# ankur-maximos/Sparse_Matrix_with_Flops

Measured on AMD Instinct MI355X. Metric: SpGEMM GFLOP/s (2*intermediate_nnz/sec), C=A*A on 1M-row CSR, higher is better.
Workload: dtype f32; 1 GPU; synthetic power-law CSR 1048576^2, ~16 nnz/row, seed 43, C=A*A; m=1048576, nnzA=15623432, intermediate_nnz_P=238121643, nnzC=226057055, bytes_alg=3971793112, parallelism=single GPU

## Files before the change

### include/spgemm_hip.h

```cpp
#ifndef SPGEMM_HIP_H_
#define SPGEMM_HIP_H_

#include <stddef.h>

#ifdef __cplusplus
extern "C" {
#endif

#define SPGEMM_OK                0
#define SPGEMM_ERR_HIP           1
#define SPGEMM_ERR_ARG           2
#define SPGEMM_ERR_OVERFLOW      3
#define SPGEMM_ERR_NOMEM         4
#define SPGEMM_ERR_INPUT         5
#define SPGEMM_ERR_INTERNAL      6
#define SPGEMM_ERR_NODEVICE      7

#define SPGEMM_NBINS             9
#define SPGEMM_HV_LEN            9
#define SPGEMM_NKERNELS          21

typedef struct spgemm_handle spgemm_handle;

typedef struct spgemm_stats {
// ... 61 lines not shown
                       const int* dIA, const int* dJA, const float* dA, int nnzA,
                       const int* dIB, const int* dJB, const float* dB, int nnzB,
                       int m, int k, int n, const int* dIC, int* dJC, float* dC);

int hip_csr_row_flops(spgemm_handle* h, const int* dIA, const int* dJA, const int* dIB, int m,
                      int* dRowFlops, long long* total_flops);

int hip_gpuFlopsClassify(spgemm_handle* h,
                         const int* dIA, const int* dJA, const int* dIB,
                         int m, int k,
                         int** drowIds, int** dflops, int hv[SPGEMM_HV_LEN], int* hv_len,
                         long long* total_flops);

int hip_sgpuSpMM(spgemm_handle* h,
                 const int* dIA, const int* dJA, const float* dA, int nnzA,
                 const int* dIB, const int* dJB, const float* dB, int nnzB,
                 int m, int k, int n,
                 const int* drowIds, const int hv[SPGEMM_HV_LEN], const int* dflops,
                 int** dIC, int** dJC, float** dC, int* nnzC);

int hip_rmcl_prune(spgemm_handle* h, int m, const int* dIC, const int* dJC, float* dC,
                   int** dIN, int** dJN, float** dCN, int* nnzN);
int hip_rmcl_prune_n(spgemm_handle* h, int m, int nnz, const int* dIC, const int* dJC, const float* dC,
                     int** dIN, int** dJN, float** dCN, int* nnzN);
int hip_rmcl_expand_prune(spgemm_handle* h,
                          const int* dIA, const int* dJA, const float* dA, int nnzA,
                          const int* dIB, const int* dJB, const float* dB, int nnzB,
                          int m, int k, int n,
                          int** dIN, int** dJN, float** dCN, int* nnzN);
int hip_gpuRmclIter_device(spgemm_handle* h, int maxIter, int rows, int cols,
                           const int* dgI, const int* dgJ, const float* dgA, int gnnz,
                           const int* dtI, const int* dtJ, const float* dtA, int tnnz,
                           int** oI, int** oJ, float** oA, int* onnz);
int hip_gpuRmclIter(int maxIter, int rows, int cols,
                    const int* gIA, const int* gJA, const float* gA, int gnnz,
                    const int* tIA, const int* tJA, const float* tA, int tnnz,
                    int** oIA, int** oJA, float** oA, int* onnz);

#define SPGEMM_XCHG_AUTO  0
#define SPGEMM_XCHG_RCCL  1
#define SPGEMM_XCHG_PEER  2
#define SPGEMM_XCHG_HOST  3
#define SPGEMM_UNIQUE_ID_BYTES 128
typedef struct spgemm_group spgemm_group;
typedef struct spgemm_sharded spgemm_sharded;
int spgemm_hip_group_create(spgemm_group** g, int nshards, const int* devices, int transport);
int spgemm_hip_rccl_available(void);
int spgemm_hip_unique_id(void* id128);
int spgemm_hip_group_create_rank(spgemm_group** g, int nranks, int rank, int device, const void* id128);
int spgemm_hip_group_info(const spgemm_group* g, int* nranks, int* nlocal, int* transport);
int spgemm_hip_group_destroy(spgemm_group* g);

int hip_sharded_spmm_create(spgemm_group* g, const int* IA, const int* JA, const float* A, int nnzA,
                            const int* IB, const int* JB, const float* B, int nnzB, int m, int k, int n,
                            spgemm_sharded** job);
int hip_sharded_spmm_step(spgemm_sharded* job, int gather, long long* nnzC, long long* totalP);
int hip_sharded_spmm_result(spgemm_sharded* job, int local_shard, int** IC, int** JC, float** C, int* nnzC, int* rows);
int hip_sharded_spmm_info(spgemm_sharded* job, int* ends, float* ms_compute, float* ms_exchange);
spgemm_handle* hip_sharded_spmm_handle(spgemm_sharded* job, int local_shard);
int hip_sharded_spmm_destroy(spgemm_sharded* job);

int hip_gpuRmclIter_sharded(spgemm_group* g, int maxIter, int rows, int cols,
                            const int* gIA, const int* gJA, const float* gA, int gnnz,
                            const int* tIA, const int* tJA, const float* tA, int tnnz,
                            int** oIA, int** oJA, float** oA, int* onnz);

typedef struct spgemm_sharded_rmcl spgemm_sharded_rmcl;
int hip_sharded_rmcl_create(spgemm_group* g, int rows, int cols, const int* gIA, const int* gJA, const float* gA, int gnnz,
                            const int* tIA, const int* tJA, const float* tA, int tnnz, spgemm_sharded_rmcl** job);
int hip_sharded_rmcl_run(spgemm_sharded_rmcl* job, int maxIter, int* nnz);
int hip_sharded_rmcl_continue(spgemm_sharded_rmcl* job, int iters, int* nnz);
int hip_sharded_rmcl_result(spgemm_sharded_rmcl* job, int local_shard, int** oIA, int** oJA, float** oA, int* onnz);
int hip_sharded_rmcl_iter_nnz(const spgemm_sharded_rmcl* job, long long* out, int cap);
int hip_sharded_rmcl_info(const spgemm_sharded_rmcl* job, int* ends);
int hip_sharded_rmcl_destroy(spgemm_sharded_rmcl* job);

int spgemm_hip_handle_device(const spgemm_handle* h);

int spgemm_hip_rmcl_devices_used(void);

int spgemm_hip_debug_fail_next(spgemm_handle* h, int count);

int spgemm_hip_debug_bigrow_paths(spgemm_handle* h, int* direct_rows, int* fallback_rows, int* rehit_cap, int* region_ints);

#define SPGEMM_COO_DEDUPE         1
#define SPGEMM_COO_SELF_LOOPS     2
#define SPGEMM_COO_ROW_NORMALISE  4
#define SPGEMM_COO_ABS            8
int hip_coo_to_csr(spgemm_handle* h, int rows, int cols, int nnz, const int* dRow, const int* dCol, const float* dVal,
                   int flags, int** dIA, int** dJA, float** dA, int* nnzOut);

#define SPGEMM_EDGES_ONE_BASED 1
#define SPGEMM_EDGES_TRANSPOSE 2
typedef struct spgemm_edge_stats {
  long long lines;
  long long first_bad_line;
  int entries, slow_lines;
  float ms_upload, ms_split, ms_parse, ms_slow, ms_total;
} spgemm_edge_stats;

int hip_edge_text_header(const char* text, size_t nbytes, int* rows, int* cols, int* declared,
                         int* one_based, int* symmetric, size_t* data_offset);
int hip_parse_edge_lines(spgemm_handle* h, const char* dText, size_t nbytes, int declared, int flags,
                         int** dRow, int** dCol, float** dVal, int* entries, spgemm_edge_stats* st);
int hip_parse_edge_text (spgemm_handle* h, const char* text,  size_t nbytes, int declared, int flags,
                         int** dRow, int** dCol, float** dVal, int* entries, spgemm_edge_stats* st);
int hip_read_edge_file  (spgemm_handle* h, const char* path, int isTrans, int cooFlags, int* rows, int* cols,
                         int** dIA, int** dJA, float** dA, int* nnz, spgemm_edge_stats* st);

#define SPGEMM_STATS_LEN 13
int hip_flopsStats(spgemm_handle* h, const int* dIA, const int* dJA, const int* dIB, int m, int stats[SPGEMM_STATS_LEN]);

#define SPGEMM_NNZ_STATS_LEN 18
int hip_nnzStats(spgemm_handle* h, const int* dIA, int m, int stats[SPGEMM_NNZ_STATS_LEN]);

typedef struct spgemm_bin_report {
  int rows;
  int rows_differ;
  int first_bad_row;
  double max_rel_err;
} spgemm_bin_report;
int hip_resultsComparison(int m, int n, const int* hIC, const int* hJC, const float* hC,
                          const int* rIC, const int* rJC, const float* rC,
                          const int hv[SPGEMM_HV_LEN], int hv_len, const int* hqueue, double rel,
                          spgemm_bin_report report[SPGEMM_HV_LEN - 1]);

int hip_csr_sort_rows(spgemm_handle* h, int m, const int* dIC, int* dJC, float* dC);

int hip_csr_permute(spgemm_handle* h, int m, int n, int nnz, const int* dIA, const int* dJA, const float* dA,
                    const int* dRowSrc, const int* dColMap, int** dIB, int** dJB, float** dB);
int hip_csr_permute_f64(spgemm_handle* h, int m, int n, int nnz, const int* dIA, const int* dJA, const double* dA,
                        const int* dRowSrc, const int* dColMap, int** dIB, int** dJB, double** dB);

int hip_permutation_transpose(spgemm_handle* h, int len, const int* dP, int* dPt);

int hip_csr_row_descending_permutation(spgemm_handle* h, int m, const int* dIA, int** dP);

int hip_csr_transpose(spgemm_handle* h, int m, int n, int nnz, const int* dIA, const int* dJA, const float* dA,
                      int** dIT, int** dJT, float** dAT);
int hip_csr_transpose_f64(spgemm_handle* h, int m, int n, int nnz, const int* dIA, const int* dJA, const double* dA,
                          int** dIT, int** dJT, double** dAT);

typedef struct spgemm_csr_diff {
  int       rows_len_differ;
  int       first_len_row;
  long long only_a, only_b;
  int       first_only_row;
  long long beyond;
  int       first_beyond_row;
  double    max_abs_err;
  double    max_rel_err;
  double    max_abs_only_a, max_abs_only_b;
  double    sum_sq;
} spgemm_csr_diff;
int hip_csr_diff(spgemm_handle* h, int m, int n,
                 const int* dIA, const int* dJA, const float* dA, int nnzA,
                 const int* dIB, const int* dJB, const float* dB, int nnzB,
                 double rel_tol, double abs_tol, spgemm_csr_diff* out);
int hip_csr_diff_f64(spgemm_handle* h, int m, int n,
                     const int* dIA, const int* dJA, const double* dA, int nnzA,
                     const int* dIB, const int* dJB, const double* dB, int nnzB,
                     double rel_tol, double abs_tol, spgemm_csr_diff* out);

int hip_csr_differsStats(spgemm_handle* h, int m, const int* dIA, const int* dIB,
                         const float* percents, int npercents, int* counts);
int hip_csr_differsStats_f64(spgemm_handle* h, int m, const int* dIA, const int* dIB,
// ... 72 lines not shown
```

### sparse_matrix_with_flops_amd/csrc/spgemm_device.hpp

```cpp
#pragma once
#include <hip/hip_runtime.h>
#include <stdint.h>
#include <type_traits>

namespace smf {

#ifdef SMF_ABLATE
__device__ int g_ablate = 0;
#define ABL(bit) (g_ablate & (bit))
__device__ __forceinline__ void smf_or(int*, int) {}
__device__ __forceinline__ void smf_or(unsigned* p, unsigned v) { atomicOr(p, v); }
#define atomicOr(p, v) smf_or((p), (v))
#else
#define ABL(bit) 0
#endif

constexpr int WAVE = 64;

template <class T> __device__ __forceinline__ void st_out(T* p, T v) {
#ifdef SMF_PLAIN_STORES
  *p = v;
#else
  __builtin_nontemporal_store(v, p);
#endif
// ... 27 lines not shown
  while (lg < 12 + NSUB - 1 && (f >> (lg + 1)) != 0) ++lg;
  return SLOT_BIG0 + (NSUB - 1 - (lg - 12));
}
__host__ __device__ __forceinline__ int last_slot_of_bin(int b) {
  return b < 5 ? b : b == 5 ? SLOT_H1B : b == 6 ? SLOT_H4B : b == 7 ? SLOT_H8 : NSLOTS - 1;
}

constexpr int ERRF_TABLE_FULL = 1;
constexpr int ERRF_COUNT_MISMATCH = 2;

__device__ __forceinline__ int lane_id() { return (int)__lane_id(); }

__device__ __forceinline__ unsigned long long ballot64(bool pred) { return __builtin_amdgcn_ballot_w64(pred); }

__device__ __forceinline__ int mask_rank(unsigned long long mask) {
  return (int)__builtin_amdgcn_mbcnt_hi((unsigned)(mask >> 32), __builtin_amdgcn_mbcnt_lo((unsigned)mask, 0u));
}

#define SMF_DPP(v, ctrl, rowmask, ident) __builtin_amdgcn_update_dpp((ident), (v), (ctrl), (rowmask), 0xf, false)

__device__ __forceinline__ int wave_incl_add(int v) {
  v += SMF_DPP(v, 0x111, 0xf, 0);
  v += SMF_DPP(v, 0x112, 0xf, 0);
  v += SMF_DPP(v, 0x114, 0xf, 0);
  v += SMF_DPP(v, 0x118, 0xf, 0);
  v += SMF_DPP(v, 0x142, 0xa, 0);
  v += SMF_DPP(v, 0x143, 0xc, 0);
  return v;
}

__device__ __forceinline__ int wave_incl_max(int v) {
  v = max(v, SMF_DPP(v, 0x111, 0xf, 0));
  v = max(v, SMF_DPP(v, 0x112, 0xf, 0));
  v = max(v, SMF_DPP(v, 0x114, 0xf, 0));
  v = max(v, SMF_DPP(v, 0x118, 0xf, 0));
  v = max(v, SMF_DPP(v, 0x142, 0xa, 0));
  v = max(v, SMF_DPP(v, 0x143, 0xc, 0));
  return v;
}

__device__ __forceinline__ int wave_sum(int v) { return __builtin_amdgcn_readlane(wave_incl_add(v), 63); }

__device__ __forceinline__ unsigned long long wave_sum_u64(unsigned long long v) {
#pragma unroll
  for (int d = 32; d >= 1; d >>= 1) v += __shfl_xor(v, d, 64);
  return v;
}

__device__ __forceinline__ void wave_lds_sync() {
  __builtin_amdgcn_fence(__ATOMIC_ACQ_REL, "wavefront");
  __builtin_amdgcn_s_waitcnt(0xc07f);
  __builtin_amdgcn_wave_barrier();
}

__device__ __forceinline__ int next_pow2_clamped(int x, int lo, int hi) {
  int p = lo;
  while (p < x && p < hi) p <<= 1;
  return p;
}

__device__ __forceinline__ int log2_pow2(int p) { return 31 - __clz(p); }

template <int MULT = 2>
__device__ __forceinline__ int table_size(int items, int lo, int hi) {
  return items >= hi / MULT ? hi : next_pow2_clamped(MULT * items, lo, hi);
}

__device__ __forceinline__ int hash_insert(int* keys, int size, int shift, int c, bool* is_new, int* err) {
  unsigned h = ((unsigned)c * 2654435761u) >> shift;
  const unsigned mask = (unsigned)size - 1u;
  *is_new = false;
  for (int probe = 0; probe < size; ++probe) {
    const int old = atomicCAS(&keys[h], EMPTY_KEY, c);
    if (old == EMPTY_KEY) { *is_new = true; return (int)h; }
    if (old == c) return (int)h;
    h = (h + 1u) & mask;
  }
  atomicOr(err, ERRF_TABLE_FULL);
  return 0;
}

constexpr int DUMMY_KEY = (int)0x80000000;

template <bool POW2 = true, int U>
__device__ __forceinline__ int hash_insert_multi(int* keys, int size, int shift, const bool (&act)[U],
                                                 const int (&col)[U], int* dummy, int* err) {
  char* const base = reinterpret_cast<char*>(keys);
  const int dumB = (int)(reinterpret_cast<char*>(dummy) - base);
  const int maskB = size * 4 - 1;
  int hB[U];
  int claimed = 0;
#pragma unroll
  for (int u = 0; u < U; ++u) {
    const unsigned hv = (unsigned)col[u] * 2654435761u;
    const unsigned h = POW2 ? hv >> shift : __umulhi(hv, (unsigned)size);
    hB[u] = act[u] ? (int)(h * 4u) : dumB;
  }
  int probe = 0;
  for (;;) {
    int old[U];
#pragma unroll
    for (int u = 0; u < U; ++u) old[u] = atomicCAS(reinterpret_cast<int*>(base + hB[u]), EMPTY_KEY, col[u]);
    ++probe;
    int pendBits = 0;
#pragma unroll
    for (int u = 0; u < U; ++u) {
      claimed += old[u] == EMPTY_KEY ? 1 : 0;
      const bool adv = hB[u] != dumB && old[u] != EMPTY_KEY && old[u] != col[u];
      const int nh = POW2 ? ((hB[u] + probe * 4) & maskB) : (hB[u] + 4 == size * 4 ? 0 : hB[u] + 4);
      hB[u] = adv ? nh : dumB;
      pendBits |= hB[u] ^ dumB;
    }
    if (ballot64(pendBits != 0) == 0ull) break;
    if (probe >= size) { atomicOr(err, ERRF_TABLE_FULL); break; }
  }
  return claimed;
}

typedef unsigned long long slot_t;
constexpr slot_t EMPTY_SLOT = 0x00000000FFFFFFFFull;
constexpr slot_t DUMMY_SLOT = 0x0000000080000000ull;
__device__ __forceinline__ slot_t make_slot(int col, float v) {
  return (slot_t)(unsigned)col | ((slot_t)__float_as_uint(v) << 32);
}
__device__ __forceinline__ int slot_key(slot_t sl) { return (int)(unsigned)sl; }
__device__ __forceinline__ float slot_val(slot_t sl) { return __uint_as_float((unsigned)(sl >> 32)); }
__device__ __forceinline__ float* slot_val_ptr(slot_t* tab, unsigned i) { return reinterpret_cast<float*>(tab + i) + 1; }

__device__ __forceinline__ void hash_accum(slot_t* tab, int size, int shift, int c, float v, int* err) {
  unsigned h = ((unsigned)c * 2654435761u) >> shift;
  const unsigned mask = (unsigned)size - 1u;
  const slot_t mine = make_slot(c, v);
  for (int probe = 0; probe < size; ++probe) {
    const slot_t old = atomicCAS(&tab[h], EMPTY_SLOT, mine);
    if (old == EMPTY_SLOT) return;
    if (slot_key(old) == c) { atomicAdd(slot_val_ptr(tab, h), v); return; }
    h = (h + 1u) & mask;
  }
  atomicOr(err, ERRF_TABLE_FULL);
}

template <bool POW2 = true, int U>
__device__ __forceinline__ void hash_accum_multi(slot_t* tab, int size, int shift, const bool (&act)[U],
                                                 const int (&col)[U], const float (&val)[U], slot_t* dummy, int* err) {
  char* const base = reinterpret_cast<char*>(tab);
  const int dumB = (int)(reinterpret_cast<char*>(dummy) - base);
  const int maskB = size * 8 - 1, sizeB = size * 8;
  int hB[U], stepB[U], dupB[U];
  slot_t mine[U];
#pragma unroll
  for (int u = 0; u < U; ++u) {
    const unsigned hv = (unsigned)col[u] * 2654435761u;
    const unsigned h = POW2 ? hv >> shift : __umulhi(hv, (unsigned)size);
    stepB[u] = POW2 ? 0 : (int)((0x2f2b29251f1d1713ull >> (((hv >> 7) & 7u) * 8u)) & 0xffu) * 8;
    hB[u] = act[u] ? (int)(h * 8u) : dumB;
    dupB[u] = dumB;
    mine[u] = make_slot(col[u], val[u]);
  }
  int probe = 0;
  for (;;) {
    slot_t old[U];
#pragma unroll
    for (int u = 0; u < U; ++u) old[u] = atomicCAS(reinterpret_cast<slot_t*>(base + hB[u]), EMPTY_SLOT, mine[u]);
    ++probe;
    int pendBits = 0;
#pragma unroll
    for (int u = 0; u < U; ++u) {
      const bool pend = hB[u] != dumB;
      const bool same = pend && slot_key(old[u]) == col[u];
      const bool adv = pend && old[u] != EMPTY_SLOT && slot_key(old[u]) != col[u];
      dupB[u] = same ? hB[u] : dupB[u];
      int nh;
      if (POW2) nh = (hB[u] + probe * 8) & maskB;
      else { nh = hB[u] + stepB[u]; nh = nh >= sizeB ? nh - sizeB : nh; }
      hB[u] = adv ? nh : dumB;
      pendBits |= hB[u] ^ dumB;
    }
    if (ballot64(pendBits != 0) == 0ull) break;
    if (probe >= size) { atomicOr(err, ERRF_TABLE_FULL); break; }
  }
#pragma unroll
  for (int u = 0; u < U; ++u)
    if (dupB[u] != dumB) atomicAdd(reinterpret_cast<float*>(base + dupB[u] + 4), val[u]);
}

template <int U>
__device__ __forceinline__ void lds_fadd_multi(float* acc, const int (&idx)[U], const bool (&ok)[U], const float (&v)[U],
                                               int* dummy) {
  int* ia = reinterpret_cast<int*>(acc);
  int old[U];
  bool pend[U];
#pragma unroll
  for (int u = 0; u < U; ++u) { pend[u] = ok[u]; old[u] = ia[ok[u] ? idx[u] : 0]; }
  for (;;) {
    int got[U];
#pragma unroll
    for (int u = 0; u < U; ++u)
      got[u] = atomicCAS(pend[u] ? &ia[idx[u]] : dummy, old[u], __float_as_int(__int_as_float(old[u]) + v[u]));
    bool more = false;
#pragma unroll
    for (int u = 0; u < U; ++u) {
      pend[u] = pend[u] && got[u] != old[u];
      old[u] = got[u];
      more = more || pend[u];
    }
    if (ballot64(more) == 0ull) break;
  }
}

template <int NW> struct InsChunk { static constexpr int value = NW == 1 ? 1 : 0; };
template <int CH, int R>
__device__ __forceinline__ int hash_insert_chunked(int* keys, int size, int shift, const bool (&act)[R], const int (&col)[R],
                                                   int* dummy, int* err) {
  if constexpr (CH <= 0 || CH >= R) return hash_insert_multi(keys, size, shift, act, col, dummy, err);
  else {
    int claimed = 0;
#pragma unroll
    for (int c0 = 0; c0 < R; c0 += CH) {
      bool a_[CH]; int c_[CH];
#pragma unroll
      for (int u = 0; u < CH; ++u) { a_[u] = c0 + u < R ? act[c0 + u < R ? c0 + u : 0] : false; c_[u] = col[c0 + u < R ? c0 + u : 0]; }
      if (CH == 1 && ballot64(a_[0]) == 0ull) continue;
      claimed += hash_insert_multi(keys, size, shift, a_, c_, dummy, err);
    }
    return claimed;
  }
}
template <int CH, int R>
__device__ __forceinline__ void hash_accum_chunked(slot_t* tab, int size, int shift, const bool (&act)[R], const int (&col)[R],
                                                   const float (&val)[R], slot_t* dummy, int* err) {
  if constexpr (CH <= 0 || CH >= R) hash_accum_multi(tab, size, shift, act, col, val, dummy, err);
  else {
#pragma unroll
    for (int c0 = 0; c0 < R; c0 += CH) {
      bool a_[CH]; int c_[CH]; float v_[CH];
#pragma unroll
      for (int u = 0; u < CH; ++u) {
        const int i = c0 + u < R ? c0 + u : 0;
        a_[u] = c0 + u < R ? act[i] : false; c_[u] = col[i]; v_[u] = val[i];
      }
      if (CH == 1 && ballot64(a_[0]) == 0ull) continue;
      hash_accum_multi(tab, size, shift, a_, c_, v_, dummy, err);
    }
  }
}

__device__ __forceinline__ void clear_slots(slot_t* tab, int size, int tid, int nthreads) {
  for (int i = tid * 2; i < size; i += nthreads * 2) *reinterpret_cast<ulonglong2*>(tab + i) = make_ulonglong2(EMPTY_SLOT, EMPTY_SLOT);
}

__device__ __forceinline__ void clear_table(int* keys, float* vals, int size, int tid, int nthreads) {
  const int4 ek = make_int4(EMPTY_KEY, EMPTY_KEY, EMPTY_KEY, EMPTY_KEY);
  const float4 zv = make_float4(0.f, 0.f, 0.f, 0.f);
  for (int i = tid * 4; i < size; i += nthreads * 4) {
    *reinterpret_cast<int4*>(keys + i) = ek;
    if (vals) *reinterpret_cast<float4*>(vals + i) = zv;
  }
}

template <int MAXSTEPS>
__device__ __forceinline__ void emit_claimed(const slot_t* tab, int base, int per, int* emitted,
                                             int outLo, int outHi, int* __restrict__ JC, float* __restrict__ C) {
  const int lane = lane_id();
  slot_t sl[MAXSTEPS];
  int cnt = 0;
#pragma unroll
  for (int sidx = 0; sidx < MAXSTEPS; ++sidx) {
    sl[sidx] = sidx * WAVE < per ? tab[base + sidx * WAVE + lane] : EMPTY_SLOT;
    cnt += __popcll(ballot64(slot_key(sl[sidx]) != EMPTY_KEY));
  }
  int pos = 0;
  if (lane == 0) pos = atomicAdd(emitted, cnt);
  pos = __builtin_amdgcn_readfirstlane(pos);
  int* const JCrow = JC + outLo;
  float* const Crow = C + outLo;
  const unsigned lim = (unsigned)(outHi - outLo);
#pragma unroll
  for (int sidx = 0; sidx < MAXSTEPS; ++sidx) {
    const bool occ = slot_key(sl[sidx]) != EMPTY_KEY;
    const unsigned long long mk = ballot64(occ);
    const unsigned o = (unsigned)(pos + mask_rank(mk));
    if (occ && o < lim) { st_out(JCrow + o, slot_key(sl[sidx])); st_out(Crow + o, slot_val(sl[sidx])); }
    pos += __popcll(mk);
  }
}

__device__ __forceinline__ float rmcl_threshold(float avg, float mx) {
  float ret = (float)(0.90 * avg * (1 - 2 * (mx - avg)));
  ret = (float)((ret > 1.0e-7) ? ret : 1.0e-7);
  ret = (ret > mx) ? mx : ret;
  return ret;
}

template <class Op>
__device__ __forceinline__ float row16_allreduce(float v, Op op) {
  v = op(v, __int_as_float(SMF_DPP(__float_as_int(v), 0xB1, 0xf, 0)));
  v = op(v, __int_as_float(SMF_DPP(__float_as_int(v), 0x4E, 0xf, 0)));
  v = op(v, __int_as_float(SMF_DPP(__float_as_int(v), 0x141, 0xf, 0)));
  v = op(v, __int_as_float(SMF_DPP(__float_as_int(v), 0x140, 0xf, 0)));
  return v;
}
template <int L, class Op>
__device__ __forceinline__ float rowL_allreduce(float v, Op op) {
  static_assert(L == 16 || L == 64, "16-lane groups or whole waves");
  v = row16_allreduce(v, op);
  if (L == 64) {
// ... 677 lines not shown
    const int sIncl = wave_incl_add(ntg), lIncl = wave_incl_add(lug);
    const int S = __builtin_amdgcn_readlane(sIncl, 63);
    const int total = S + __builtin_amdgcn_readlane(lIncl, 63);
    int tIncl = 0, lpIncl = 0, gLPv = 0, shortSum = 0;
    if (num) {
      gLPv = lane < NW ? num->gLP[lane] : 0;
      tIncl = wave_incl_add(gT);
      lpIncl = wave_incl_add(gLPv);
      shortSum = __builtin_amdgcn_readlane(tIncl, 63);
    }
    for (int u = __builtin_amdgcn_readfirstlane(w); u < total;) {
      int unext = 0;
      if (lane == 0) unext = atomicAdd(&st.claim, 1);
      if (u < S) {
        const int g = __popcll(ballot64(sIncl <= u));
        const int t = u - (__builtin_amdgcn_readlane(sIncl, g) - __builtin_amdgcn_readlane(ntg, g));
        const int T = __builtin_amdgcn_readlane(gT, g), ns = __builtin_amdgcn_readlane(gNS, g);
        unsigned long long W[U];
        int base[U];
#pragma unroll
        for (int uu = 0; uu < U; ++uu) {
          const int r = min(t * U + uu, WAVE - 1);
          W[uu] = st.marks[g][r];
          base[uu] = st.wpre[g][r];
        }
        const int p0 = num ? chunkBase + (__builtin_amdgcn_readlane(tIncl, g) - T) + t * U * WAVE : -1;
        short_trip<U, NEED_VAL, 16>(reinterpret_cast<const char*>(st.rec[g]), T, ns, t * U, W, base, JB, VB, f, p0);
      } else {
        const int ul = u - S;
        const int g = __popcll(ballot64(lIncl <= ul));
        const int ug = ul - (__builtin_amdgcn_readlane(lIncl, g) - __builtin_amdgcn_readlane(lug, g));
        const int nl = __builtin_amdgcn_readlane(gNL, g);
        const int uex = lane < nl ? st.rec[g][WAVE - 1 - lane].w : 0x7fffffff;
        const int k = __popcll(ballot64(uex <= ug)) - 1;
        const int4 r4 = st.rec[g][WAVE - 1 - k];
        const int p0 = num ? chunkBase + shortSum + (__builtin_amdgcn_readlane(lpIncl, g) - __builtin_amdgcn_readlane(gLPv, g)) +
                                 num->lpro[g][k] + (ug - r4.w) * UP
                           : -1;
        long_trip<U, NEED_VAL>(r4.x, r4.z, __int_as_float(r4.y), (ug - r4.w) * UP, JB, VB, f, p0);
      }
      u = __builtin_amdgcn_readfirstlane(unext);
    }
    __builtin_amdgcn_s_waitcnt(0xc07f);
    if (num) chunkBase += shortSum + __builtin_amdgcn_readlane(lpIncl, 63);
    __syncthreads();
  }
}

template <int R>
__device__ __forceinline__ int next_row(int* ctr, int* slot, int prev) {
  if (R > 1 && prev >= 0 && (prev + 1) % R != 0) return prev + 1;
  if (threadIdx.x == 0) *slot = atomicAdd(ctr, R);
  __syncthreads();
  const int q = *slot;
  __syncthreads();
  return q;
}
__device__ __forceinline__ int next_row(int* ctr, int* slot) { return next_row<1>(ctr, slot, -1); }

struct RowMeta { int row, as, ae, x0, x1, x2; };

__device__ __forceinline__ RowMeta load_meta_sym(const int* rows, int q, int count, const int* IA, const int* rowFlops) {
  RowMeta mtd{0, 0, 0, 0, 0, 0};
  if (q < count) { mtd.row = rows[q]; mtd.as = IA[mtd.row]; mtd.ae = IA[mtd.row + 1]; mtd.x0 = rowFlops[mtd.row]; }
  return mtd;
}
__device__ __forceinline__ RowMeta load_meta_num(const int* rows, int q, int count, const int* IA, const int* IC,
                                                 const int* rowFlops = nullptr) {
  RowMeta mtd{0, 0, 0, 0, 0, 0};
  if (q < count) {
    mtd.row = rows[q]; mtd.as = IA[mtd.row]; mtd.ae = IA[mtd.row + 1]; mtd.x0 = IC[mtd.row]; mtd.x1 = IC[mtd.row + 1];
    if (rowFlops) mtd.x2 = rowFlops[mtd.row];
  }
  return mtd;
}

__device__ __forceinline__ PreA load_pre(const RowMeta& mtd, const int2* SBL, const float* VA, bool needVal) {
  PreA p{0, 0, 0.f, true};
  const int ap = mtd.as + lane_id();
  if (ap < mtd.ae) { const int2 sbl = SBL[ap]; p.bs = sbl.x; p.len = sbl.y; if (needVal) p.a = VA[ap]; }
  return p;
}

template <int NW, int TBL, int U>
__global__ __launch_bounds__(WAVE * NW) void k_sym_hash(const int* __restrict__ binPtr, int bin,
                                                         const int* __restrict__ rowIds,
                                                         const int* __restrict__ IA, const int2* __restrict__ SBL,
                                                         const int* __restrict__ JB,
                                                         const int* __restrict__ rowFlops, int* __restrict__ IC,
                                                         int* __restrict__ err, int* __restrict__ qctr) {
  __shared__ __attribute__((aligned(16))) int keys[TBL];
  __shared__ typename WalkSel<NW>::type st;
  __shared__ int cnt_s;
  __shared__ int qslot;
  const int tid = threadIdx.x, lane = lane_id();
  if (tid < WAVE) st.dummy[tid] = DUMMY_SLOT;
  int first = binPtr[bin], count = binPtr[bin + 1] - first;
  constexpr int QB = NW >= 8 ? 2 : 4;
  int stride = (int)gridDim.x;
  if (NW == 1) {
    const XcdRange xr = xcd_range(count);
    first += xr.lo; count = xr.hi - xr.lo; stride = xr.nb;
  }
  const int* rows = rowIds + first;
  int q = NW > 1 ? next_row<QB>(qctr, &qslot, -1) : (int)(blockIdx.x >> 3);
  RowMeta cur = load_meta_sym(rows, q, count, IA, rowFlops);
  RowMeta nxt = NW == 1 ? load_meta_sym(rows, q + stride, count, IA, rowFlops) : RowMeta{0, 0, 0, 0, 0, 0};
  PreA pc = NW == 1 ? load_pre(cur, SBL, nullptr, false) : PreA{0, 0, 0.f, false};
  while (q < count) {
    int qn;
    PreA pn{0, 0, 0.f, false};
    RowMeta nn{0, 0, 0, 0, 0};
    if (NW == 1) {
      qn = q + stride;
      nn = load_meta_sym(rows, qn + stride, count, IA, rowFlops);
      pn = load_pre(nxt, SBL, nullptr, false);
    } else {
      qn = next_row<QB>(qctr, &qslot, q);
      nxt = load_meta_sym(rows, qn, count, IA, rowFlops);
    }
    const int size = table_size<4>(cur.x0, 64, TBL);
    const int shift = 32 - log2_pow2(size);
    clear_table(keys, nullptr, size, tid, WAVE * NW);
    if (tid == 0) cnt_s = 0;
    __syncthreads();
    int mine = 0;
    for_each_product<NW, U, false>(st, cur.as, cur.ae, SBL, nullptr, JB, nullptr,
                                   [&](const auto& act, const auto& col, const auto& val, int) {
      mine += hash_insert_chunked<InsChunk<NW>::value>(keys, size, shift, act, col, reinterpret_cast<int*>(&st.dummy[lane_id()]), err);
    }, pc, err);
    const int ws = wave_sum(mine);
    if (NW == 1) {
      if (lane == 0) IC[cur.row] = ws;
    } else {
      if (lane == 0 && ws) atomicAdd(&cnt_s, ws);
      __syncthreads();
      if (tid == 0) IC[cur.row] = cnt_s;
    }
    __syncthreads();
    cur = nxt;
    if (NW == 1) { nxt = nn; pc = pn; }
    q = qn;
  }
}

template <int NW, int TBL, int U, int PRUNE = 0>
__global__ __launch_bounds__(WAVE * NW) void k_num_hash(const int* __restrict__ binPtr, int bin,
                                                         const int* __restrict__ rowIds,
                                                         const int* __restrict__ IA, const int2* __restrict__ SBL,
                                                         const float* __restrict__ VA,
                                                         const int* __restrict__ JB,
                                                         const float* __restrict__ VB,
                                                         const int* __restrict__ IC, int* __restrict__ JC,
                                                         float* __restrict__ C, int* __restrict__ err,
                                                         int* __restrict__ qctr, const int* __restrict__ rowFlops,
                                                         int* __restrict__ pcnt) {
  __shared__ __attribute__((aligned(16))) slot_t tab[TBL];
  __shared__ PruneShared<NW> ps;
  __shared__ typename WalkSel<NW>::type st;
  __shared__ int qslot;
  __shared__ int emitted;
  const int tid = threadIdx.x;
  if (tid < WAVE) st.dummy[tid] = DUMMY_SLOT;
  constexpr int T = WAVE * NW;
  int first = binPtr[bin], count = binPtr[bin + 1] - first;
  constexpr int QB = NW >= 8 ? 2 : 4;
  int stride = (int)gridDim.x;
  if (NW == 1) {
    const XcdRange xr = xcd_range(count);
    first += xr.lo; count = xr.hi - xr.lo; stride = xr.nb;
  }
  const int* rows = rowIds + first;
  int q = NW > 1 ? next_row<QB>(qctr, &qslot, -1) : (int)(blockIdx.x >> 3);
  const int* const rf = rowFlops;
  RowMeta cur = load_meta_num(rows, q, count, IA, IC, rf);
  RowMeta nxt = NW == 1 ? load_meta_num(rows, q + stride, count, IA, IC, rf) : RowMeta{0, 0, 0, 0, 0, 0};
  PreA pc = NW == 1 ? load_pre(cur, SBL, VA, true) : PreA{0, 0, 0.f, false};
  while (q < count) {
    int qn;
    PreA pn{0, 0, 0.f, false};
    RowMeta nn{0, 0, 0, 0, 0};
    if (NW == 1) {
      qn = q + stride;
      nn = load_meta_num(rows, qn + stride, count, IA, IC, rf);
      pn = load_pre(nxt, SBL, VA, true);
    } else {
      qn = next_row<QB>(qctr, &qslot, q);
      nxt = load_meta_num(rows, qn, count, IA, IC, rf);
    }
    const int off = cur.x0;
    const int want = cur.x1 - off;
    if (NW == 1 && PRUNE == 1 && want == cur.x2 && want <= TBL) {
      for_each_product<NW, U, true>(st, cur.as, cur.ae, SBL, VA, JB, VB,
                                    [&](const auto& act, const auto& col, const auto& val, int p0) {
        constexpr int R = (int)(sizeof(col) / sizeof(col[0]));
#pragma unroll
        for (int u = 0; u < R; ++u) {
          const unsigned o = (unsigned)(p0 + u * WAVE + lane_id());
          if (act[u] && o < (unsigned)want) tab[o] = make_slot(col[u], val[u]);
        }
      }, pc, err);
      wave_lds_sync();
      int nocc;
      const int kept = prune_emit_group<64>(tab, (want + 63) & ~63, want, false, true, lane_id(), JC + off, C + off, &nocc);
      if (lane_id() == 0) pcnt[cur.row] = kept;
      wave_lds_sync();
      cur = nxt;
      nxt = nn; pc = pn;
      q = qn;
      continue;
    }
    if (NW == 1 && PRUNE == 0 && want == cur.x2) {
      int* const JCrow = JC + off;
      float* const Crow = C + off;
      for_each_product<NW, U, true>(st, cur.as, cur.ae, SBL, VA, JB, VB,
                                    [&](const auto& act, const auto& col, const auto& val, int p0) {
        constexpr int R = (int)(sizeof(col) / sizeof(col[0]));
#pragma unroll
        for (int u = 0; u < R; ++u) {
          const unsigned o = (unsigned)(p0 + u * WAVE + lane_id());
          if (act[u] && o < (unsigned)want) { st_out(JCrow + o, col[u]); st_out(Crow + o, val[u]); }
        }
      }, pc, err);
      cur = nxt;
      if (NW == 1) { nxt = nn; pc = pn; }
      q = qn;
// ... 565 lines not shown
      clear_slots(sh.tab, size, tid, T);
      if (tid == 0) sh.emitted = 0;
      __syncthreads();
      {
        const int* const lg = rlLog + cur.ls;
        const unsigned mask = (unsigned)size - 1u;
        for (int i = tid; i < lc; i += T) {
          const int c = lg[i];
          const slot_t mine = make_slot(c, -0.0f);
          unsigned h = ((unsigned)c * 2654435761u) >> shift;
          for (int probe = 0; probe < size; ++probe) {
            const slot_t old = atomicCAS(&sh.tab[h], EMPTY_SLOT, mine);
            if (old == EMPTY_SLOT || slot_key(old) == c) break;
            h = (h + 1u) & mask;
          }
        }
      }
      __syncthreads();
      int* const JCrow = JC + outBase;
      float* const Crow = C + outBase;
      const unsigned lim = (unsigned)max(want, 0);
      for_each_product<NW, BD_U, true>(sh.st, as, ae, SBL, VA, JB, VB,
                                       [&](const bool (&act)[BD_U], const int (&col)[BD_U], const float (&val)[BD_U], int) {
        char* const base = reinterpret_cast<char*>(sh.tab);
        const int dumB = (int)(reinterpret_cast<char*>(&sh.st.dummy[lane]) - base);
        const int maskB = size * 8 - 1;
        int hB[BD_U], hitB[BD_U];
        bool miss[BD_U];
#pragma unroll
        for (int u = 0; u < BD_U; ++u) {
          const unsigned h = ((unsigned)col[u] * 2654435761u) >> shift;
          hB[u] = act[u] ? (int)(h * 8u) : dumB;
          hitB[u] = dumB;
          miss[u] = false;
        }
        for (int probe = 0;;) {
          int key[BD_U];
#pragma unroll
          for (int u = 0; u < BD_U; ++u) key[u] = *reinterpret_cast<const int*>(base + hB[u]);
          ++probe;
          int pendBits = 0;
#pragma unroll
          for (int u = 0; u < BD_U; ++u) {
            const bool pend = hB[u] != dumB;
            const bool hit = pend && key[u] == col[u];
            const bool emp = pend && key[u] == EMPTY_KEY;
            hitB[u] = hit ? hB[u] : hitB[u];
            miss[u] = miss[u] || emp;
            hB[u] = (pend && !hit && !emp) ? ((hB[u] + 8) & maskB) : dumB;
            pendBits |= hB[u] ^ dumB;
          }
          if (ballot64(pendBits != 0) == 0ull) break;
          if (probe >= size) { atomicOr(err, ERRF_TABLE_FULL); break; }
        }
#pragma unroll
        for (int u = 0; u < BD_U; ++u)
          if (hitB[u] != dumB) atomicAdd(reinterpret_cast<float*>(base + hitB[u] + 4), val[u]);
        unsigned long long mk[BD_U];
        int tot = 0;
#pragma unroll
        for (int u = 0; u < BD_U; ++u) { mk[u] = ballot64(miss[u]); tot += __popcll(mk[u]); }
        if (tot) {
          int pos = 0;
          if (lane == 0) pos = atomicAdd(&sh.emitted, tot);
          pos = __builtin_amdgcn_readfirstlane(pos);
#pragma unroll
          for (int u = 0; u < BD_U; ++u) {
            const unsigned o = (unsigned)(pos + mask_rank(mk[u]));
            if (miss[u] && o < lim) { st_out(JCrow + o, col[u]); st_out(Crow + o, val[u]); }
            pos += __popcll(mk[u]);
          }
        }
      });
      emit_claimed<S / NW / WAVE>(sh.tab, w * per, per, &sh.emitted, outBase, outEnd, JC, C);
      __syncthreads();
      if (tid == 0 && sh.emitted != want) atomicOr(err, ERRF_COUNT_MISMATCH);
      __syncthreads();
    }
    cur = nxt;
    q = qn;
  }
}

constexpr int SCAN_THREADS = 1024;
constexpr int SCAN_ITEMS = 4;
constexpr int SCAN_TILE = SCAN_THREADS * SCAN_ITEMS;

__global__ __launch_bounds__(SCAN_THREADS) void k_scan_tile_sums(int m, const int* __restrict__ IC,
                                                                  unsigned long long* __restrict__ tileSum) {
  __shared__ unsigned long long red[16];
  const int tid = threadIdx.x, lane = lane_id(), w = tid >> 6;
  const int base = blockIdx.x * SCAN_TILE + tid * SCAN_ITEMS;
  unsigned long long s = 0;
#pragma unroll
  for (int i = 0; i < SCAN_ITEMS; ++i) if (base + i < m) s += (unsigned)IC[base + i];
  s = wave_sum_u64(s);
  if (lane == 0) red[w] = s;
  __syncthreads();
  if (tid == 0) { unsigned long long t = 0; for (int i = 0; i < 16; ++i) t += red[i]; tileSum[blockIdx.x] = t; }
}

__global__ __launch_bounds__(1024) void k_scan_tiles(int ntiles, unsigned long long* __restrict__ tileSum,
                                                      unsigned long long* __restrict__ total) {
  __shared__ unsigned long long wsum[16];
  __shared__ unsigned long long running;
  const int tid = threadIdx.x, lane = lane_id(), w = tid >> 6;
  if (tid == 0) running = 0;
  __syncthreads();
  for (int t0 = 0; t0 < ntiles; t0 += 1024) {
    const int t = t0 + tid;
    const unsigned long long v = t < ntiles ? tileSum[t] : 0ull;
    unsigned long long incl = v;
#pragma unroll
    for (int d = 1; d < 64; d <<= 1) { const unsigned long long o = __shfl_up(incl, d, 64); if (lane >= d) incl += o; }
    if (lane == 63) wsum[w] = incl;
    __syncthreads();
    unsigned long long woff = 0, tot = 0;
    for (int i = 0; i < 16; ++i) { const unsigned long long s = wsum[i]; tot += s; if (i < w) woff += s; }
    const unsigned long long run = running;
    if (t < ntiles) tileSum[t] = run + woff + incl - v;
    __syncthreads();
    if (tid == 0) running = run + tot;
    __syncthreads();
  }
  if (tid == 0) *total = running;
}

__global__ __launch_bounds__(SCAN_THREADS) void k_scan_apply(int m, int* __restrict__ IC,
                                                              const unsigned long long* __restrict__ tileOff,
                                                              const unsigned long long* __restrict__ total, int clampTotal) {
  __shared__ int wsum[16];
  const int tid = threadIdx.x, lane = lane_id(), w = tid >> 6;
  const int base = blockIdx.x * SCAN_TILE + tid * SCAN_ITEMS;
  int v[SCAN_ITEMS];
  int s = 0;
#pragma unroll
  for (int i = 0; i < SCAN_ITEMS; ++i) { v[i] = base + i < m ? IC[base + i] : 0; s += v[i]; }
  const int incl = wave_incl_add(s);
  if (lane == 63) wsum[w] = incl;
  __syncthreads();
  int woff = 0;
  for (int i = 0; i < w; ++i) woff += wsum[i];
  int run = (int)tileOff[blockIdx.x] + woff + incl - s;
#pragma unroll
  for (int i = 0; i < SCAN_ITEMS; ++i) { if (base + i < m) IC[base + i] = run; run += v[i]; }
  if (blockIdx.x == 0 && tid == 0) {
    const unsigned long long t = *total;
    IC[m] = (clampTotal && t > 0x7fffffffULL) ? 0x7fffffff : (int)(unsigned)t;
  }
}

__global__ void k_gather_flops(int m, const int* __restrict__ rowIds, const int* __restrict__ rowFlops,
                               int* __restrict__ out) {
  const int q = blockIdx.x * blockDim.x + threadIdx.x;
  if (q < m) out[q] = rowFlops[rowIds[q]];
}

constexpr int SORT_MAX = 4096;
template <class V>
__global__ __launch_bounds__(256) void k_sort_rows(int m, const int* __restrict__ IC, int* __restrict__ JC,
                                                    V* __restrict__ C, int* __restrict__ longUnsorted) {
  __shared__ int sk[SORT_MAX];
  __shared__ V sv[SORT_MAX];
  __shared__ int unsorted;
  const int tid = threadIdx.x;
  for (int row = blockIdx.x; row < m; row += gridDim.x) {
// ... 272 lines not shown
```

### sparse_matrix_with_flops_amd/csrc/spgemm_hip.hip

```cpp
#include "spgemm_device.hpp"
#include "spgemm_f64_device.hpp"
#include "chain_device.hpp"
#include "../../include/spgemm_hip.h"

#include <algorithm>
#include <array>
#include <chrono>
#include <climits>
#include <cmath>
#include <cstdarg>
#include <cstdio>
#include <cstdlib>
#include <cstring>
#include <map>
#include <mutex>
#include <sys/mman.h>
#include <thread>
#include <type_traits>
#include <vector>

using namespace smf;

static_assert(NBINS == SPGEMM_NBINS, "bin count of the kernels and of the C ABI differ");
#ifdef SMF_ABLATE
// ... 68 lines not shown
    return e;
  }
  hipError_t release(void* p) {
    if (!p) return hipSuccess;
    if (check) (void)hipDeviceSynchronize();
    Blk blk{0, 0};
    {
      std::lock_guard<std::mutex> lk(mu);
      auto it = live.find(p);
      if (it == live.end()) return hipFree(p);
      blk = it->second;
      live.erase(it);
      if (cached_bytes + blk.size <= kMaxCached) {
        free_blocks[blk.dev].emplace(blk.size, p);
        cached_bytes += blk.size;
        return hipSuccess;
      }
    }
    return hipFree(p);
  }
  void trim(int dev) {
    std::lock_guard<std::mutex> lk(mu);
    auto& fb = free_blocks[dev];
    for (auto& kv : fb) { cached_bytes -= kv.first; (void)hipFree(kv.second); }
    fb.clear();
  }
  size_t cached_on(int dev) {
    std::lock_guard<std::mutex> lk(mu);
    size_t t = 0;
    for (auto& kv : free_blocks[dev]) t += kv.first;
    return t;
  }
};
DevPool& pool() { static DevPool* p = new DevPool(); return *p; }

template <class T>
struct DevBuf {
  T* p = nullptr;
  DevBuf() = default;
  DevBuf(DevBuf&& o) noexcept : p(o.release()) {}
  DevBuf& operator=(DevBuf&& o) noexcept { if (this != &o) { reset(); p = o.release(); } return *this; }
  ~DevBuf() { reset(); }
  hipError_t alloc(size_t n) { reset(); return pool().alloc((void**)&p, sizeof(T) * n); }
  void reset() { pool().release(p); p = nullptr; }
  T* release() { T* q = p; p = nullptr; return q; }
  operator T*() const { return p; }
};

struct CsrView {
  const int* I; const int* J; const float* V; int nnz;
  const int* len = nullptr; const int2* se = nullptr;
};

struct DevCSR {
  DevBuf<int> I, J; DevBuf<float> V; DevBuf<int> len; DevBuf<int2> se;
  int rows = 0, cols = 0, nnz = 0;
  bool packed() const { return !len; }
  CsrView view() const { return {I, J, V, nnz, len, se}; }
  hipError_t alloc_entries(long long n) {
    const hipError_t e = J.alloc((size_t)std::max(n, 1ll));
    return e != hipSuccess ? e : V.alloc((size_t)std::max(n, 1ll));
  }
  void reset() { *this = DevCSR(); }
  void give(int** oI, int** oJ, float** oV, int* onnz) {
    *oI = I.release(); *oJ = J.release(); *oV = V.release(); *onnz = nnz;
    reset();
  }
};

static int drained(hipStream_t s, int rc) {
  if (rc) (void)hipStreamSynchronize(s);
  return rc;
}
struct Retired {
  DevCSR m;
  void park(DevCSR&& operand) { m = std::move(operand); }
};
}

struct HostMirror {
  int binPtr[NBINS + 1];
  int err;
  int scratch2[4];
  alignas(128) int qctr[9 * 32];
  alignas(128) int qpad_;
  int slotBase[NSLOTS + 1];
  unsigned long long totalP;
  unsigned long long nnzC64;
  unsigned long long kept64;
  unsigned long long cutTotal;
  int nBatches;
  alignas(128) int chainTicket;
  alignas(128) int chainPad_;
  alignas(128) int fbBin[2];
  alignas(128) int fbPad_;
};

struct spgemm_handle {
  int device = 0;
  int numCU = 256;
  hipStream_t stream = nullptr;
  hipEvent_t ev[6] = {nullptr, nullptr, nullptr, nullptr, nullptr, nullptr};
  int cap_m = -1;
  int* rowFlops = nullptr;
  unsigned char* binId = nullptr;
  int* blockHist = nullptr;
  int* blockOff = nullptr;
  int* rowIds = nullptr;
  unsigned long long* tileSum = nullptr;
  unsigned long long* blockP = nullptr;
  int2* sbl = nullptr;
  int* batchStart = nullptr;
  unsigned long long* chainWords = nullptr;
  int pathMode = 0;
  int chainCfg = 0;
  long long cap_nnz = -1;
  HostMirror* dsmall = nullptr;
  HostMirror* hsmall = nullptr;
  HostMirror mirror;
  const int* cur_rowIds = nullptr;
  int sym_m = -1;
  hipEvent_t kev[2 * SPGEMM_NKERNELS];
  bool kused[SPGEMM_NKERNELS];
  unsigned ktiming = 0;
  hipEvent_t evMid = nullptr;
  HostMirror* hmid = nullptr;
  static constexpr int NSIDE = 4;
  hipStream_t side[NSIDE] = {nullptr, nullptr, nullptr, nullptr};
  hipEvent_t fork_ev = nullptr;
  hipEvent_t join_ev[NSIDE] = {nullptr, nullptr, nullptr, nullptr};
  bool serial = true;
  int U = 2;
  unsigned* bigBitmaps = nullptr;
  int bm_cap = 0;
  int2* spill = nullptr;
  int spill_blocks = 0;
  int bhCap = BH_CAP;
  int bhMargin = 125;
  bool bigDirect = true;
  int bdCfg = 1;
  int bdMinRows = 0;
  int rlRegionEnv = 0;
  int2* rlMeta = nullptr;
  int rl_rows = 0;
  int* rlLog = nullptr;
  int rl_region = 0;
  int* bigFallback = nullptr;
  bool bdLogged = false;
  bool bdRan = false;
  int h1sym = 32;
  int h1num = 24;
  spgemm_stats stats;
  spgemm_host_api_stats host_api = {};
  int failNext = 0;
  int prev_m = -1;
  unsigned long long prev_P = 0;
  long long prev_nnzC = -1;
};

static std::mutex g_count_mu;
static std::map<int, int> g_handles_on;

struct WsBlock { void** ptr; size_t bytes; };
static std::array<WsBlock, 10> ws_blocks(spgemm_handle* h, size_t cap) {
  const size_t nblk = (cap + K1_THREADS - 1) / K1_THREADS;
  const size_t ntile = (cap + 1 + SCAN_TILE - 1) / SCAN_TILE + 1;
  return {{{(void**)&h->rowFlops, sizeof(int) * cap},
           {(void**)&h->binId, cap},
           {(void**)&h->blockHist, sizeof(int) * nblk * NSLOTS},
           {(void**)&h->blockOff, sizeof(int) * nblk * NSLOTS},
           {(void**)&h->rowIds, sizeof(int) * cap},
           {(void**)&h->tileSum, sizeof(unsigned long long) * ntile},
           {(void**)&h->blockP, sizeof(unsigned long long) * nblk},
           {(void**)&h->bigFallback, sizeof(int) * cap},
           {(void**)&h->batchStart, sizeof(int) * (3 * cap + 64)},
           {(void**)&h->chainWords, sizeof(unsigned long long) * (3 * cap + 64)}}};
}

static int ws_free(spgemm_handle* h) {
  for (const WsBlock& b : ws_blocks(h, 0)) { hipFree(*b.ptr); *b.ptr = nullptr; }
  h->cap_m = -1;
  return SPGEMM_OK;
}

static int ws_ensure_entries(spgemm_handle* h, long long nnzA) {
  if (nnzA <= h->cap_nnz) return SPGEMM_OK;
  hipFree(h->sbl);
  h->sbl = nullptr; h->cap_nnz = -1;
  const long long cap = nnzA + nnzA / 8 + 1024;
  HIPCHK(hipMalloc((void**)&h->sbl, sizeof(int2) * (size_t)cap));
  h->cap_nnz = cap;
  return SPGEMM_OK;
}

static int ws_ensure(spgemm_handle* h, int m) {
  if (m <= h->cap_m) return SPGEMM_OK;
  ws_free(h);
  const size_t cap = (size_t)m + (size_t)m / 8 + 1024;
  for (const WsBlock& b : ws_blocks(h, cap)) HIPCHK(hipMalloc(b.ptr, b.bytes));
  h->cap_m = (int)std::min<size_t>(cap, 0x7fffffff);
  return SPGEMM_OK;
}

template <class F>
static auto with_bd_cfg(int cfg, F f) {
  typedef std::integral_constant<int, 4> W4; typedef std::integral_constant<int, 8> W8; typedef std::integral_constant<int, 16> W16;
  typedef std::integral_constant<int, 4096> S4; typedef std::integral_constant<int, 8192> S8;
  switch (cfg) {
    case 0: return f(W4(), S4());
    case 1: return f(W8(), S4());
    case 2: return f(W4(), S8());
    case 4: return f(W16(), S4());
    default: return f(W8(), S8());
  }
}
static int bd_cap_of(int cfg) { return bd_cap(cfg == 2 || cfg == 3 ? 8192 : 4096); }

static void env_int(const char* name, int lo, int hi, int* field) {
  if (const char* e = getenv(name)) { const int v = atoi(e); if (v >= lo && v <= hi) *field = v; }
}

extern "C" int spgemm_hip_device_count(int* count) {
  if (!count) return fail(SPGEMM_ERR_ARG, "count is null");
  int n = 0;
  hipError_t e = hipGetDeviceCount(&n);
  if (e != hipSuccess) { *count = 0; return fail(SPGEMM_ERR_NODEVICE, "hipGetDeviceCount: %s", hipGetErrorString(e)); }
  *count = n;
  return SPGEMM_OK;
}

extern "C" int spgemm_hip_create(spgemm_handle** out, int device) {
  if (!out) return fail(SPGEMM_ERR_ARG, "handle out-pointer is null");
  *out = nullptr;
  int n = 0;
  if (hipGetDeviceCount(&n) != hipSuccess || n <= 0)
    return fail(SPGEMM_ERR_NODEVICE, "no HIP device visible: libspgemm_hip has no CPU fallback");
  if (device < 0 || device >= n) return fail(SPGEMM_ERR_ARG, "device %d out of range [0,%d)", device, n);
  HIPCHK(hipSetDevice(device));
  spgemm_handle* h = new spgemm_handle();
  h->device = device;
  hipDeviceProp_t prop;
  HIPCHK(hipGetDeviceProperties(&prop, device));
  h->numCU = prop.multiProcessorCount > 0 ? prop.multiProcessorCount : 256;
  HIPCHK(hipStreamCreateWithFlags(&h->stream, hipStreamNonBlocking));
  for (auto& e : h->ev) HIPCHK(hipEventCreate(&e));
  for (auto& e : h->kev) HIPCHK(hipEventCreate(&e));
  for (auto& u : h->kused) u = false;
  { const char* e = getenv("SPGEMM_CONCURRENT"); h->serial = !(e && e[0] == '1'); }
#ifdef SMF_ABLATE
  { int v = 0; env_int("SPGEMM_ABLATE", INT_MIN, INT_MAX, &v); HIPCHK(hipMemcpyToSymbol(HIP_SYMBOL(smf::g_ablate), &v, sizeof(int))); }
#endif
  env_int("SPGEMM_H1SYM", 1, 32, &h->h1sym);
  env_int("SPGEMM_H1NUM", 1, 32, &h->h1num);
  env_int("SPGEMM_BHMARGIN", 10, 400, &h->bhMargin);
  env_int("SPGEMM_BHCAP", 1024, BH_CAP_MAX, &h->bhCap);
  { int v = 1; env_int("SPGEMM_BIGDIRECT", 0, 1, &v); h->bigDirect = v != 0; }
  env_int("SPGEMM_BD_CFG", 0, 4, &h->bdCfg);
  h->bdMinRows = h->numCU;
  env_int("SPGEMM_BD_MINROWS", 1, 1 << 30, &h->bdMinRows);
  env_int("SPGEMM_RLREGION", 64, 1 << 24, &h->rlRegionEnv);
  env_int("SPGEMM_PATH", 0, 2, &h->pathMode);
  env_int("SPGEMM_CHAIN_CFG", INT_MIN, INT_MAX, &h->chainCfg);
  { int u = h->U; env_int("SPGEMM_U", 2, 8, &u); if (u == 2 || u == 4 || u == 8) h->U = u; }
  for (auto& st : h->side) {
    if (h->serial) st = h->stream;
    else HIPCHK(hipStreamCreateWithFlags(&st, hipStreamNonBlocking));
  }
  HIPCHK(hipEventCreateWithFlags(&h->fork_ev, hipEventDisableTiming));
  for (auto& e : h->join_ev) HIPCHK(hipEventCreateWithFlags(&e, hipEventDisableTiming));
  HIPCHK(hipMalloc((void**)&h->dsmall, sizeof(HostMirror)));
  HIPCHK(hipHostMalloc((void**)&h->hsmall, sizeof(HostMirror), hipHostMallocDefault));
  HIPCHK(hipHostMalloc((void**)&h->hmid, sizeof(HostMirror), hipHostMallocDefault));
  HIPCHK(hipEventCreateWithFlags(&h->evMid, hipEventDisableTiming));
  { const char* e = getenv("SPGEMM_KTIMING"); if (e) h->ktiming = (unsigned)strtoul(e, nullptr, 0); }
  memset(&h->stats, 0, sizeof(h->stats));
  { std::lock_guard<std::mutex> lk(g_count_mu); ++g_handles_on[device]; }
  HIPCHK(hipFuncSetAttribute((const void*)k_sym_big<false>, hipFuncAttributeMaxDynamicSharedMemorySize, (int)sizeof(BigSymShared)));
  HIPCHK(hipFuncSetAttribute((const void*)k_sym_big<true>, hipFuncAttributeMaxDynamicSharedMemorySize, (int)sizeof(BigSymShared)));
  HIPCHK(with_bd_cfg(h->bdCfg, [&](auto nw, auto slots) {
    return hipFuncSetAttribute((const void*)k_num_bigdirect<nw, slots>, hipFuncAttributeMaxDynamicSharedMemorySize,
                               (int)sizeof(BigDirectShared<nw, slots>)); }));
  HIPCHK(hipFuncSetAttribute((const void*)k_num_big, hipFuncAttributeMaxDynamicSharedMemorySize, (int)sizeof(BigNumShared)));
  HIPCHK(hipFuncSetAttribute((const void*)k_num_bighash, hipFuncAttributeMaxDynamicSharedMemorySize, (int)sizeof(BigHashShared)));
  *out = h;
  return SPGEMM_OK;
}

extern "C" int spgemm_hip_destroy(spgemm_handle* h) {
  if (!h) return SPGEMM_OK;
  hipSetDevice(h->device);
  if (h->stream) hipStreamSynchronize(h->stream);
  for (auto& st : h->side) if (st && st != h->stream) { hipStreamSynchronize(st); hipStreamDestroy(st); }
  ws_free(h);
  hipFree(h->bigBitmaps);
  hipFree(h->spill);
  hipFree(h->rlMeta);
  hipFree(h->rlLog);
  hipFree(h->sbl);
  hipFree(h->dsmall);
  hipHostFree(h->hsmall);
  hipHostFree(h->hmid);
  if (h->evMid) hipEventDestroy(h->evMid);
  for (auto& e : h->ev) if (e) hipEventDestroy(e);
  for (auto& e : h->kev) if (e) hipEventDestroy(e);
  if (h->fork_ev) hipEventDestroy(h->fork_ev);
  for (auto& e : h->join_ev) if (e) hipEventDestroy(e);
  if (h->stream) hipStreamDestroy(h->stream);
  bool last = false;
  { std::lock_guard<std::mutex> lk(g_count_mu); last = --g_handles_on[h->device] <= 0; }
  if (last) pool().trim(h->device);
  delete h;
  return SPGEMM_OK;
}

extern "C" int spgemm_hip_get_stats(const spgemm_handle* h, spgemm_stats* out) {
  if (!h || !out) return fail(SPGEMM_ERR_ARG, "null argument");
  *out = h->stats;
  return SPGEMM_OK;
}

extern "C" void* spgemm_hip_stream(spgemm_handle* h) { return h ? (void*)h->stream : nullptr; }

extern "C" int spgemm_hip_handle_device(const spgemm_handle* h) { return h ? h->device : -1; }

extern "C" int spgemm_hip_debug_bigrow_paths(spgemm_handle* h, int* direct_rows, int* fallback_rows, int* rehit_cap, int* region_ints) {
  if (!h || !direct_rows || !fallback_rows || !rehit_cap || !region_ints) return fail(SPGEMM_ERR_ARG, "null argument");
  const int nbig = h->mirror.binPtr[NBINS] - h->mirror.binPtr[NBINS - 1];
  *fallback_rows = h->bdRan ? h->mirror.fbBin[1] : nbig;
  *direct_rows = nbig - *fallback_rows;
  *rehit_cap = bd_cap_of(h->bdCfg);
  *region_ints = h->rl_region;
  return SPGEMM_OK;
}

extern "C" int spgemm_hip_debug_fail_next(spgemm_handle* h, int count) {
  if (!h) return fail(SPGEMM_ERR_ARG, "null handle");
  h->failNext = count;
  return SPGEMM_OK;
}

extern "C" int spgemm_hip_set_kernel_timing(spgemm_handle* h, unsigned mask) {
  if (!h) return fail(SPGEMM_ERR_ARG, "null handle");
  h->ktiming = mask;
  return SPGEMM_OK;
}

static std::mutex g_default_mu;
static spgemm_handle* g_default = nullptr;
static int default_handle(spgemm_handle** out) {
  std::lock_guard<std::mutex> lk(g_default_mu);
  if (!g_default) CHK(spgemm_hip_create(&g_default, 0));
  *out = g_default;
  return SPGEMM_OK;
}

extern "C" int spgemm_hip_malloc(void** dptr, size_t bytes) {
  if (!dptr) return fail(SPGEMM_ERR_ARG, "dptr is null");
  *dptr = nullptr;
  HIPCHK(pool().alloc(dptr, bytes ? bytes : 1));
  return SPGEMM_OK;
}
extern "C" int spgemm_hip_pool_cached_bytes(int device, size_t* bytes) {
  if (!bytes) return fail(SPGEMM_ERR_ARG, "bytes is null");
  *bytes = pool().cached_on(device);
  return SPGEMM_OK;
}
extern "C" int spgemm_hip_pool_trim(int device) {
  int n = 0;
  if (hipGetDeviceCount(&n) != hipSuccess || device < 0 || device >= n) return fail(SPGEMM_ERR_ARG, "device %d out of range", device);
  int cur = 0;
  const bool had = hipGetDevice(&cur) == hipSuccess;
  HIPCHK(hipSetDevice(device));
  pool().trim(device);
  if (had) (void)hipSetDevice(cur);
  return SPGEMM_OK;
}
extern "C" int spgemm_hip_free(void* dptr) {
  HIPCHK(pool().release(dptr));
  return SPGEMM_OK;
}
struct CopyJob { void* host; void* dev; size_t bytes; };
static int copy_pageable(int dev, const CopyJob* jobs, int njobs, bool toDevice);
static constexpr size_t kLaneCopyMin = size_t(8) << 20;
static int device_of(const void* dptr) {
  hipPointerAttribute_t a;
  if (hipPointerGetAttributes(&a, dptr) == hipSuccess) return a.device;
  (void)hipGetLastError();
  int dev = 0;
  (void)hipGetDevice(&dev);
  return dev;
}

extern "C" int spgemm_hip_memcpy_h2d(void* dst, const void* src, size_t bytes) {
  if (bytes && (!dst || !src)) return fail(SPGEMM_ERR_ARG, "null pointer in h2d copy");
  if (bytes >= kLaneCopyMin) {
    const CopyJob j{const_cast<void*>(src), dst, bytes};
    return copy_pageable(device_of(dst), &j, 1, true);
  }
  if (bytes) HIPCHK(hipMemcpy(dst, src, bytes, hipMemcpyHostToDevice));
  return SPGEMM_OK;
}
extern "C" int spgemm_hip_memcpy_d2h(void* dst, const void* src, size_t bytes) {
  if (bytes && (!dst || !src)) return fail(SPGEMM_ERR_ARG, "null pointer in d2h copy");
  if (bytes >= kLaneCopyMin) {
    const CopyJob j{dst, const_cast<void*>(src), bytes};
    return copy_pageable(device_of(src), &j, 1, false);
  }
  if (bytes) HIPCHK(hipMemcpy(dst, src, bytes, hipMemcpyDeviceToHost));
  return SPGEMM_OK;
}

extern "C" int spgemm_hip_memcpy_d2d(void* dst, const void* src, size_t bytes) {
  if (bytes && (!dst || !src)) return fail(SPGEMM_ERR_ARG, "null pointer in d2d copy");
  if (bytes) HIPCHK(hipMemcpy(dst, src, bytes, hipMemcpyDeviceToDevice));
// ... 16 lines not shown
    "k_num_hash<1,1024>", "k_num_hash<4,4096>", "k_num_hash<8,8192>", "k_num_big", "k_num_bighash", "k_cut(3 launches)",
    "k_chain", "k_wbatch<sym>", "k_wbatch<num>"};
extern "C" const char* spgemm_hip_kernel_name(int id) { return (id >= 0 && id < SPGEMM_NKERNELS) ? kKernelNames[id] : ""; }

struct KTimer {
  spgemm_handle* h; int id; hipStream_t s; bool on;
  KTimer(spgemm_handle* h_, int id_, hipStream_t s_ = nullptr)
      : h(h_), id(id_), s(s_ ? s_ : h_->stream), on((h_->ktiming >> id_) & 1u) {
    if (on) { hipEventRecord(h->kev[2 * id], s); h->kused[id] = true; }
  }
  ~KTimer() { if (on) hipEventRecord(h->kev[2 * id + 1], s); }
};

static void collect_kernel_times(spgemm_handle* h, bool reset) {
  for (int i = 0; i < SPGEMM_NKERNELS; ++i) {
    if (reset) h->stats.ms_kernel[i] = 0.f;
    if (h->kused[i]) { float ms = 0.f; if (hipEventElapsedTime(&ms, h->kev[2 * i], h->kev[2 * i + 1]) == hipSuccess) h->stats.ms_kernel[i] = ms; }
    h->kused[i] = false;
  }
}

static void fork_streams(spgemm_handle* h) {
  if (h->serial) return;
  hipEventRecord(h->fork_ev, h->stream);
  for (auto& st : h->side) hipStreamWaitEvent(st, h->fork_ev, 0);
}
static void join_streams(spgemm_handle* h) {
  if (h->serial) return;
  for (int i = 0; i < spgemm_handle::NSIDE; ++i) {
    hipEventRecord(h->join_ev[i], h->side[i]);
    hipStreamWaitEvent(h->stream, h->join_ev[i], 0);
  }
}

#define LAUNCH_U(KERN, NW, TBL, grid, block, st, ...)                                              \
  do {                                                                                             \
    if (h->U == 8) hipLaunchKernelGGL((KERN<NW, TBL, 8>), grid, block, 0, st, __VA_ARGS__);        \
    else if (h->U == 4) hipLaunchKernelGGL((KERN<NW, TBL, 4>), grid, block, 0, st, __VA_ARGS__);   \
    else hipLaunchKernelGGL((KERN<NW, TBL, 2>), grid, block, 0, st, __VA_ARGS__);                  \
  } while (0)

template <class F>
static void with_prune_arg(const int* pcnt, int pmode, F f) {
  if (pcnt && pmode == 2) f(std::integral_constant<int, 2>());
  else if (pcnt) f(std::integral_constant<int, 1>());
  else f(std::integral_constant<int, 0>());
}

#define LAUNCH_NUM(NW, TBL, grid, block, st, ...)                                                                  \
  with_prune_arg(pcnt, pmode, [&](auto prune) {                                                                    \
    if constexpr (prune != 0) hipLaunchKernelGGL((k_num_hash<NW, TBL, 2, prune>), grid, block, 0, st, __VA_ARGS__, pcnt); \
    else LAUNCH_U(k_num_hash, NW, TBL, grid, block, st, __VA_ARGS__, (int*)nullptr);                               \
  })

static int launch_classify(spgemm_handle* h, const int* dIA, const int* dJA, const int* dIB, int m, long long nnzA, int* dIC,
                           const int2* dIBse = nullptr) {
  const int nblk = cdiv(m, K1_THREADS);
  clear_stale_hip_error();
  HIPCHK(hipMemsetAsync(h->dsmall, 0, sizeof(HostMirror), h->stream));
  if (nnzA >= 0) CHK(ws_ensure_entries(h, nnzA));
  if (m > 0) {
    { KTimer t(h, SPGEMM_K_ROW_FLOPS);
      int2* const sbl = nnzA >= 0 ? h->sbl : (int2*)nullptr;
      const int cap = (int)std::max(nnzA, 0ll);
      if (dIBse) hipLaunchKernelGGL(k_row_flops<true>, dim3(nblk), dim3(K1_THREADS), 0, h->stream, m, dIA, dJA, dIB, dIBse,
                                    sbl, cap, h->rowFlops, h->binId, h->blockHist, h->blockP, dIC);
      else hipLaunchKernelGGL(k_row_flops<false>, dim3(nblk), dim3(K1_THREADS), 0, h->stream, m, dIA, dJA, dIB, dIBse,
                              sbl, cap, h->rowFlops, h->binId, h->blockHist, h->blockP, dIC); }
    { KTimer t(h, SPGEMM_K_BIN_SCAN);
      hipLaunchKernelGGL(k_bin_scan, dim3(1), dim3(1024), 0, h->stream, nblk, h->blockHist, h->blockOff,
                         h->dsmall->binPtr, h->dsmall->slotBase, h->blockP, &h->dsmall->totalP); }
    { KTimer t(h, SPGEMM_K_SCATTER);
      hipLaunchKernelGGL(k_scatter_rows, dim3(nblk), dim3(K1_THREADS), 0, h->stream, m, h->binId, h->blockOff,
                         h->dsmall->slotBase, h->rowIds); }
  }
  HIPCHK(hipGetLastError());
  return SPGEMM_OK;
}

static int launch_symbolic(spgemm_handle* h, const int* dIA, const int* dJB,
                           int m, int n, const int* rowIds, int* dIC, int minBin = 0, bool skipH1A = false, bool logBig = false) {
  const int2* sbl = h->sbl;
  h->bdLogged = logBig && h->bigDirect && n > BIG_WC && m > 0;
  if (m <= 0) return SPGEMM_OK;
  clear_stale_hip_error();
  const int* bp = h->dsmall->binPtr;
  int* err = &h->dsmall->err;
  int* qc = h->dsmall->qctr;
  const int cu = h->numCU;
  fork_streams(h);
  { hipStream_t st = h->side[3]; KTimer t(h, SPGEMM_K_SYM_BIG, st);
    if (h->bdLogged)
      hipLaunchKernelGGL(k_sym_big<true>, dim3(clampi(m, 1, cu)), dim3(BIG_THREADS), sizeof(BigSymShared), st, bp, 8,
                         rowIds, dIA, sbl, dJB, n, dIC, h->bigBitmaps, h->bm_cap, qc + 0 * 32,
                         h->rlMeta, h->rlLog ? h->rl_rows : 0, h->rlLog, h->rl_region, bd_cap_of(h->bdCfg), h->bigFallback,
                         &h->dsmall->fbBin[1]);
    else
      hipLaunchKernelGGL(k_sym_big<false>, dim3(clampi(m, 1, cu)), dim3(BIG_THREADS), sizeof(BigSymShared), st, bp, 8,
                         rowIds, dIA, sbl, dJB, n, dIC, h->bigBitmaps, h->bm_cap, qc + 0 * 32,
                         (int2*)nullptr, 0, (int*)nullptr, 0, 0, (int*)nullptr, (int*)nullptr); }
  if (minBin <= 7) { hipStream_t st = h->side[2]; KTimer t(h, SPGEMM_K_SYM_HASH8, st);
    LAUNCH_U(k_sym_hash, 8, 8192, dim3(clampi(m, 1, cu * 3)), dim3(512), st, bp, 7, rowIds, dIA,
             sbl, dJB, h->rowFlops, dIC, err, qc + 1 * 32); }
  if (minBin <= 6) { hipStream_t st = h->side[2]; KTimer t(h, SPGEMM_K_SYM_HASH4, st);
    LAUNCH_U(k_sym_hash, 4, 4096, dim3(clampi(m, 1, cu * 8)), dim3(256), st, bp, 6, rowIds, dIA,
             sbl, dJB, h->rowFlops, dIC, err, qc + 2 * 32); }
  if (minBin <= 5) { hipStream_t st = h->side[1]; KTimer t(h, SPGEMM_K_SYM_HASH1, st);
    const int* sb = h->dsmall->slotBase;
    if (!skipH1A)
    LAUNCH_U(k_sym_hash, 1, 512, dim3(grid8(m, cu * h->h1sym)), dim3(64), st, sb, SLOT_H1A, rowIds, dIA,
             sbl, dJB, h->rowFlops, dIC, err, qc + 3 * 32);
    LAUNCH_U(k_sym_hash, 1, 1024, dim3(grid8(m, cu * h->h1sym)), dim3(64), st, sb, SLOT_H1B, rowIds, dIA,
             sbl, dJB, h->rowFlops, dIC, err, qc + 3 * 32); }
  if (minBin <= 4) { hipStream_t st = h->side[0]; KTimer t(h, SPGEMM_K_SYM_G16, st);
    hipLaunchKernelGGL((k_sym_g16<128, 4>), dim3(grid8(cdiv(m, 16), cu * 16)), dim3(256), 0, st, bp, 4, 5,
                       rowIds, dIA, sbl, dJB, h->rowFlops, dIC, err); }
  if (minBin <= 3) { KTimer t(h, SPGEMM_K_SYM_SMALL4);
    hipLaunchKernelGGL((k_sym_g16<32, 1>), dim3(grid8(cdiv(m, 16), cu * 16)), dim3(256), 0, h->stream, bp, 2, 4,
                       rowIds, dIA, sbl, dJB, h->rowFlops, dIC, err); }
  join_streams(h);
  HIPCHK(hipGetLastError());
  return SPGEMM_OK;
}

static int launch_scan(spgemm_handle* h, int* cnt, int m, unsigned long long* dTotal, bool clampTotal = true) {
  const int ntiles = std::max(1, cdiv(m, SCAN_TILE));
  clear_stale_hip_error();
  KTimer t(h, SPGEMM_K_SCAN);
  hipLaunchKernelGGL(k_scan_tile_sums, dim3(ntiles), dim3(SCAN_THREADS), 0, h->stream, m, cnt, h->tileSum);
  hipLaunchKernelGGL(k_scan_tiles, dim3(1), dim3(1024), 0, h->stream, ntiles, h->tileSum, dTotal);
  hipLaunchKernelGGL(k_scan_apply, dim3(ntiles), dim3(SCAN_THREADS), 0, h->stream, m, cnt, h->tileSum, dTotal, clampTotal ? 1 : 0);
  HIPCHK(hipGetLastError());
  return SPGEMM_OK;
}

static int launch_numeric(spgemm_handle* h, const int* dIA, const float* dA,
                          const int* dJB, const float* dB, int n, const int* rowIds, const int* hostBinPtr,
                          const int* dIC, int* dJC, float* dC, int* pcnt = nullptr, int pmode = 1, int minBin = 0,
                          bool skipH1A = false) {
  const int2* sbl = h->sbl;
  clear_stale_hip_error();
  const int* bp = h->dsmall->binPtr;
  int* err = &h->dsmall->err;
  int* qc = h->dsmall->qctr;
  const int cu = h->numCU;
  auto rows = [&](int lo, int hi) { return lo < minBin ? 0 : hostBinPtr[hi] - hostBinPtr[lo]; };
  fork_streams(h);
  if (rows(8, 9) > 0) {
    hipStream_t st = h->side[3];
    if (n <= BIG_WC) { KTimer t(h, SPGEMM_K_NUM_BIG, st);
      hipLaunchKernelGGL(k_num_big, dim3(clampi(rows(8, 9), 1, cu)), dim3(BIG_THREADS), sizeof(BigNumShared), st,
                         bp, 8, rowIds, dIA, sbl, dA, dJB, dB, n, dIC, dJC, dC, err, h->bigBitmaps, h->bm_cap,
                         qc + 4 * 32);
    } else { KTimer t(h, SPGEMM_K_NUM_BIGHASH, st);
      const int blocks = clampi(rows(8, 9), 1, cu);
      const bool direct = h->bdLogged && !pcnt && rows(8, 9) >= h->bdMinRows;
      h->bdRan = direct;
      if (blocks > h->spill_blocks) {
        hipFree(h->spill);
        h->spill = nullptr;
        h->spill_blocks = 0;
        if (hipMalloc((void**)&h->spill, (size_t)blocks * BH_SPILL * sizeof(int2)) == hipSuccess) h->spill_blocks = blocks;
        else (void)hipGetLastError();
      }
      hipLaunchKernelGGL(k_num_bighash, dim3(blocks), dim3(BIG_THREADS), sizeof(BigHashShared), st,
                         direct ? h->dsmall->fbBin : bp, direct ? 0 : 8, direct ? h->bigFallback : rowIds, dIA, sbl, dA, dJB,
                         dB, dIC, dJC, dC, err, qc + 4 * 32, h->rowFlops,
                         h->spill_blocks >= blocks ? h->spill : (int2*)nullptr, BH_SPILL, h->bhCap, h->bhMargin);
      if (direct && h->rlLog)
        with_bd_cfg(h->bdCfg, [&](auto nw, auto slots) {
          const int lds = (int)sizeof(BigDirectShared<nw, slots>);
          const int perCU = std::max(1, std::min((160 * 1024) / lds, 32 / (int)nw));
          hipLaunchKernelGGL((k_num_bigdirect<nw, slots>), dim3(clampi(rows(8, 9), 1, cu * perCU)), dim3(WAVE * nw), lds, st,
                             bp, 8, rowIds, dIA, sbl, dA, dJB, dB, dIC, dJC, dC, err, qc + 8 * 32,
                             (const int2*)h->rlMeta, h->rl_rows, (const int*)h->rlLog);
          return 0; }); }
    if (pcnt) hipLaunchKernelGGL(k_rmcl_fix_rows, dim3(clampi(rows(8, 9), 1, cu * 8)), dim3(256), 0, st,
                                 bp, 8, 9, rowIds, dIC, dJC, dC, pcnt);
  }
  if (rows(7, 8) > 0) { hipStream_t st = h->side[2]; KTimer t(h, SPGEMM_K_NUM_HASH8, st);
    LAUNCH_NUM(8, 8192, dim3(clampi(rows(7, 8), 1, cu * 2)), dim3(512), st, bp, 7,
             rowIds, dIA, sbl, dA, dJB, dB, dIC, dJC, dC, err, qc + 5 * 32, h->rowFlops); }
  if (rows(6, 7) > 0) { hipStream_t st = h->side[2]; KTimer t(h, SPGEMM_K_NUM_HASH4, st);
    const int* sb = h->dsmall->slotBase;
    const int* hs_ = h->mirror.slotBase;
    const int na = hs_[SLOT_H4A + 1] - hs_[SLOT_H4A], nb = hs_[SLOT_H4B + 1] - hs_[SLOT_H4B];
    if (na > 0) LAUNCH_NUM(4, 2048, dim3(clampi(na, 1, cu * 7)), dim3(256), st, sb, SLOT_H4A,
                         rowIds, dIA, sbl, dA, dJB, dB, dIC, dJC, dC, err, qc + 6 * 32, h->rowFlops);
    if (nb > 0) LAUNCH_NUM(4, 4096, dim3(clampi(nb, 1, cu * 4)), dim3(256), st, sb, SLOT_H4B,
                         rowIds, dIA, sbl, dA, dJB, dB, dIC, dJC, dC, err, qc + 7 * 32, h->rowFlops); }
  if (rows(5, 6) > 0) { hipStream_t st = h->side[1]; KTimer t(h, SPGEMM_K_NUM_HASH1, st);
    const int* sb = h->dsmall->slotBase;
    const int* hs_ = h->mirror.slotBase;
    const int na = hs_[SLOT_H1A + 1] - hs_[SLOT_H1A], nb = hs_[SLOT_H1B + 1] - hs_[SLOT_H1B];
    if (na > 0 && !skipH1A) LAUNCH_NUM(1, 512, dim3(grid8(na, cu * h->h1num)), dim3(64), st, sb, SLOT_H1A,
                         rowIds, dIA, sbl, dA, dJB, dB, dIC, dJC, dC, err, qc + 7 * 32, h->rowFlops);
    if (nb > 0) LAUNCH_NUM(1, 1024, dim3(grid8(nb, cu * 16)), dim3(64), st, sb, SLOT_H1B,
                         rowIds, dIA, sbl, dA, dJB, dB, dIC, dJC, dC, err, qc + 7 * 32, h->rowFlops); }
  if (rows(4, 5) > 0) { hipStream_t st = h->side[0]; KTimer t(h, SPGEMM_K_NUM_G16, st);
    with_prune_arg(pcnt, pmode, [&](auto prune) {
      hipLaunchKernelGGL((k_num_g16<128, 4, decltype(prune)::value>), dim3(grid8(cdiv(rows(4, 5), 16), cu * 16)), dim3(256), 0, st,
                         bp, 4, 5, rowIds, dIA, sbl, dA, dJB, dB, dIC, dJC, dC, err, h->rowFlops, pcnt); }); }
  if (minBin <= 1 && rows(1, 4) > 0) { KTimer t(h, SPGEMM_K_NUM_SMALL4);
    with_prune_arg(pcnt, pmode, [&](auto prune) {
      hipLaunchKernelGGL((k_num_g16<32, 1, decltype(prune)::value>), dim3(grid8(cdiv(rows(1, 4), 16), cu * 16)), dim3(256), 0, h->stream,
                         bp, 1, 4, rowIds, dIA, sbl, dA, dJB, dB, dIC, dJC, dC, err, h->rowFlops, pcnt); }); }
  join_streams(h);
  HIPCHK(hipGetLastError());
  return SPGEMM_OK;
}

struct ChainCfg { int nw, tbl, bpc, smallMax, minBin; bool skipH1A; };
static const ChainCfg kChainCfgs[] = {
    {4, 1280, 3, 512, 6, false},
    {6, 1280, 2, 512, 6, false},
    {4, 1024, 3, 256, 5, true},
    {4, 2048, 2, 512, 6, false},
    {8, 1280, 1, 512, 6, false},
};
static const ChainCfg& chain_cfg(const spgemm_handle* h) {
  const int n = (int)(sizeof(kChainCfgs) / sizeof(kChainCfgs[0]));
  return kChainCfgs[h->chainCfg >= 0 && h->chainCfg < n ? h->chainCfg : 0];
}
#ifndef SMF_WB_MAXR
#define SMF_WB_MAXR 2
#endif

static int launch_cut(spgemm_handle* h, int m) {
  const ChainCfg& c = chain_cfg(h);
  const int ntiles = std::max(1, cdiv(m, SCAN_TILE));
  const CutParams p{c.smallMax, c.tbl - wb_slots(c.smallMax), WAVE};
  clear_stale_hip_error();
  KTimer t(h, SPGEMM_K_CUT);
  hipLaunchKernelGGL(k_cut_sums, dim3(ntiles), dim3(SCAN_THREADS), 0, h->stream, m, h->rowFlops, p, h->tileSum);
  hipLaunchKernelGGL(k_scan_tiles, dim3(1), dim3(1024), 0, h->stream, ntiles, h->tileSum, &h->dsmall->cutTotal);
  hipLaunchKernelGGL(k_cut_apply, dim3(ntiles), dim3(SCAN_THREADS), 0, h->stream, m, h->rowFlops, p, h->tileSum,
                     h->batchStart, h->chainWords, &h->dsmall->nBatches, &h->dsmall->chainTicket);
  HIPCHK(hipGetLastError());
  return SPGEMM_OK;
}

template <int NW, int TBL, int MODE>
static void launch_wbatch_t(spgemm_handle* h, int blocks, int m, const int* dIA, const float* dA, const int* dJB, const float* dB,
                            int smallMax, int* dIC, int* dJC, float* dC, long long capC) {
  typedef WaveBatchShared<NW, TBL> Sh;
  static bool attr = false;
  if (!attr) { (void)hipFuncSetAttribute((const void*)k_wbatch<NW, TBL, MODE, SMF_WB_MAXR>, hipFuncAttributeMaxDynamicSharedMemorySize, (int)sizeof(Sh)); attr = true; }
  hipLaunchKernelGGL((k_wbatch<NW, TBL, MODE, SMF_WB_MAXR>), dim3(blocks), dim3(WAVE * NW), sizeof(Sh), h->stream, m, dIA, h->sbl, dA, dJB, dB,
                     h->rowFlops, smallMax, h->batchStart, &h->dsmall->nBatches, h->chainWords, &h->dsmall->chainTicket, dIC, dJC, dC,
                     capC, &h->dsmall->nnzC64, &h->dsmall->err);
}

template <int MODE>
static int launch_wbatch(spgemm_handle* h, int m, const int* dIA, const float* dA, const int* dJB, const float* dB,
                         int* dIC, int* dJC, float* dC, long long capC) {
  const ChainCfg& c = chain_cfg(h);
  clear_stale_hip_error();
  KTimer t(h, MODE == WB_SYM ? SPGEMM_K_WB_SYM : MODE == WB_NUM ? SPGEMM_K_WB_NUM : SPGEMM_K_CHAIN);
  const int blocks = clampi((long long)h->numCU * c.bpc, 1, 1 << 20);
  switch (h->chainCfg) {
    case 1: launch_wbatch_t<6, 1280, MODE>(h, blocks, m, dIA, dA, dJB, dB, c.smallMax, dIC, dJC, dC, capC); break;
    case 2: launch_wbatch_t<4, 1024, MODE>(h, blocks, m, dIA, dA, dJB, dB, c.smallMax, dIC, dJC, dC, capC); break;
    case 3: launch_wbatch_t<4, 2048, MODE>(h, blocks, m, dIA, dA, dJB, dB, c.smallMax, dIC, dJC, dC, capC); break;
    case 4: launch_wbatch_t<8, 1280, MODE>(h, blocks, m, dIA, dA, dJB, dB, c.smallMax, dIC, dJC, dC, capC); break;
    default: launch_wbatch_t<4, 1280, MODE>(h, blocks, m, dIA, dA, dJB, dB, c.smallMax, dIC, dJC, dC, capC); break;
  }
// ... 38 lines not shown
    st.ms_total = st.ms_classify + st.ms_symbolic + st.ms_scan_alloc;
  } else {
    hipEventElapsedTime(&st.ms_numeric, h->ev[4], h->ev[5]);
    hipEventElapsedTime(&st.ms_total, h->ev[0], h->ev[5]);
  }
  collect_kernel_times(h, true);
}

static bool fetch_mirror(spgemm_handle* h) {
  return hipMemcpyAsync(h->hsmall, h->dsmall, sizeof(HostMirror), hipMemcpyDeviceToHost, h->stream) == hipSuccess &&
         hipStreamSynchronize(h->stream) == hipSuccess;
}

static int read_mirror(spgemm_handle* h, const char* phase, int deferred = 0) {
  if (!fetch_mirror(h)) return fail(SPGEMM_ERR_HIP, "%s failed: %s", phase, hipGetErrorString(hipGetLastError()));
  h->mirror = *h->hsmall;
  const HostMirror& hm = h->mirror;
  if (hm.err && !(hm.err & deferred)) return fail(SPGEMM_ERR_INTERNAL, "device invariant broken in %s (flags=%d)", phase, hm.err);
  if (hm.nnzC64 > 0x7fffffffULL) return fail(SPGEMM_ERR_OVERFLOW, "nnz(C)=%llu does not fit int32 CSR", hm.nnzC64);
  return SPGEMM_OK;
}

static int finish_symbolic(spgemm_handle* h, int m, int* nnzCp) {
  CHK(read_mirror(h, "symbolic phase"));
  publish_stats(h, h->mirror, StatsForm::Symbolic);
  h->sym_m = m;
  *nnzCp = (int)h->mirror.nnzC64;
  return SPGEMM_OK;
}

static int symbolic_phase(spgemm_handle* h, const int* dIA, const int* dJA, int nnzA, const int* dIB, const int* dJB,
                          int m, int k, int n, const PreClass* pre, int* dIC, int* nnzCp, bool logBig = true) {
  (void)k;
  if (h->failNext > 0) { --h->failNext; return fail(SPGEMM_ERR_INTERNAL, "forced failure (spgemm_hip_debug_fail_next)"); }
  hipStream_t s = h->stream;
  hipEventRecord(h->ev[0], s);
  h->cur_rowIds = h->rowIds;
  if (pre) {
    CHK(unpack_classification(h, m, *pre, dIC));
    h->cur_rowIds = pre->drowIds;
    CHK(ws_ensure_entries(h, nnzA));
    if (nnzA > 0)
      hipLaunchKernelGGL(k_entry_lens, dim3(clampi(cdiv(nnzA, 256), 1, h->numCU * 32)), dim3(256), 0, s, nnzA, dJA, dIB, h->sbl);
  } else {
    CHK(launch_classify(h, dIA, dJA, dIB, m, nnzA, dIC));
  }
  hipEventRecord(h->ev[1], s);
  CHK(launch_symbolic(h, dIA, dJB, m, n, h->cur_rowIds, dIC, 0, false, logBig));
  hipEventRecord(h->ev[2], s);
  if (m > 0) CHK(launch_scan(h, dIC, m, &h->dsmall->nnzC64));
  else HIPCHK(hipMemsetAsync(dIC, 0, sizeof(int), s));
  hipEventRecord(h->ev[3], s);
  return finish_symbolic(h, m, nnzCp);
}

static void grow_bitmaps(spgemm_handle* h, int n) {
  const int nbig = h->mirror.binPtr[NBINS] - h->mirror.binPtr[NBINS - 1];
  if (n <= BIG_WC && nbig > h->bm_cap) {
    hipFree(h->bigBitmaps);
    h->bigBitmaps = nullptr;
    const int cap = nbig + nbig / 4 + 16;
    if (hipMalloc((void**)&h->bigBitmaps, (size_t)cap * BIG_WORDS * sizeof(unsigned)) == hipSuccess) h->bm_cap = cap;
    else { h->bm_cap = 0; (void)hipGetLastError(); }
  }
}

static void grow_rehit_log(spgemm_handle* h, int n) {
  const int nbig = h->mirror.binPtr[NBINS] - h->mirror.binPtr[NBINS - 1];
  if (!h->bigDirect || n <= BIG_WC || nbig <= h->rl_rows || nbig < h->bdMinRows) return;
  hipFree(h->rlMeta); hipFree(h->rlLog);
  h->rlMeta = nullptr; h->rlLog = nullptr; h->rl_rows = 0; h->rl_region = 0;
  const int cap = nbig + nbig / 4 + 16;
  const long long perBlock = ((long long)cap + h->numCU - 1) / h->numCU * RL_ROW_BUDGET;
  long long region = h->rlRegionEnv > 0 ? h->rlRegionEnv : std::max<long long>(RL_MIN_REGION, perBlock);
  region = std::min<long long>(region, (1ll << 30) / h->numCU);
  if (hipMalloc((void**)&h->rlMeta, (size_t)cap * sizeof(int2)) == hipSuccess &&
      hipMalloc((void**)&h->rlLog, (size_t)region * (size_t)h->numCU * sizeof(int)) == hipSuccess) {
    h->rl_rows = cap; h->rl_region = (int)region;
  } else {
    (void)hipGetLastError();
    hipFree(h->rlMeta); hipFree(h->rlLog);
    h->rlMeta = nullptr; h->rlLog = nullptr;
  }
}

static int launch_numeric_f64(spgemm_handle* h, const int* dIA, const double* dA, const int* dJB, const double* dB,
                              const int* rowIds, const int* hostBinPtr, const int* dIC, int* dJC, double* dC,
                              int** gbuf) {
  const int2* sbl = h->sbl;
  clear_stale_hip_error();
  const int* bp = h->dsmall->binPtr;
  int* err = &h->dsmall->err;
  const int cu = h->numCU;
  hipStream_t s = h->stream;
  auto rows = [&](int lo, int hi) { return hostBinPtr[hi] - hostBinPtr[lo]; };
  int wide[2] = {0, 0};
  int* gkeys = nullptr;
  double* gvals = nullptr;
  int gslots = 0, gblocks = 0;
  if (rows(8, 9) > 0) {
    int* dw = nullptr;
    HIPCHK(pool().alloc((void**)&dw, sizeof(int) * 2));
    *gbuf = dw;
    HIPCHK(hipMemsetAsync(dw, 0, sizeof(int) * 2, s));
    hipLaunchKernelGGL(k_num64_wide_rows, dim3(clampi(cdiv(rows(8, 9), 256), 1, cu)), dim3(256), 0, s, bp, 8, rowIds, dIC,
                       F64_PASS_MAXL, dw);
    if (hipMemcpyAsync(wide, dw, sizeof(wide), hipMemcpyDeviceToHost, s) != hipSuccess || hipStreamSynchronize(s) != hipSuccess)
      return fail(SPGEMM_ERR_HIP, "f64 wide-row probe failed: %s", hipGetErrorString(hipGetLastError()));
    if (wide[1] > 0) {
      gslots = 64;
      while (gslots < 2 * wide[0]) gslots <<= 1;
      const size_t perBlock = (size_t)gslots * (sizeof(int) + sizeof(double));
      gblocks = (int)std::max<size_t>(1, std::min<size_t>({(size_t)wide[1], (size_t)cu, (size_t(1) << 30) / perBlock}));
      HIPCHK(pool().alloc((void**)&gbuf[1], perBlock * (size_t)gblocks));
      gkeys = gbuf[1];
      gvals = reinterpret_cast<double*>(gkeys + (size_t)gslots * gblocks);
    }
  }
  fork_streams(h);
  if (rows(8, 9) > 0) {
    hipStream_t st = h->side[3];
    { KTimer t(h, SPGEMM_K_NUM_BIG, st);
      hipLaunchKernelGGL((k_num64_rows<F64_BIG_THREADS, F64_LDS_TBL, false>), dim3(clampi(rows(8, 9), 1, cu)),
                         dim3(F64_BIG_THREADS), 0, st, bp, 8, rowIds, dIA, sbl, dA, dJB, dB, dIC, dJC, dC, err, 0,
                         F64_PASS_MAXL, (int*)nullptr, (double*)nullptr, 0); }
    if (gblocks > 0) { KTimer t(h, SPGEMM_K_NUM_BIGHASH, st);
      hipLaunchKernelGGL((k_num64_rows<F64_BIG_THREADS, 1, true>), dim3(gblocks), dim3(F64_BIG_THREADS), 0, st, bp, 8,
                         rowIds, dIA, sbl, dA, dJB, dB, dIC, dJC, dC, err, F64_PASS_MAXL + 1, 0x7fffffff, gkeys, gvals, gslots); }
  }
  if (rows(7, 8) > 0) { hipStream_t st = h->side[2]; KTimer t(h, SPGEMM_K_NUM_HASH8, st);
    hipLaunchKernelGGL((k_num64_rows<512, 8192, false>), dim3(clampi(rows(7, 8), 1, cu)), dim3(512), 0, st, bp, 7, rowIds,
                       dIA, sbl, dA, dJB, dB, dIC, dJC, dC, err, 0, 0x7fffffff, (int*)nullptr, (double*)nullptr, 0); }
  if (rows(6, 7) > 0) { hipStream_t st = h->side[2]; KTimer t(h, SPGEMM_K_NUM_HASH4, st);
    hipLaunchKernelGGL((k_num64_rows<256, 4096, false>), dim3(clampi(rows(6, 7), 1, cu * 3)), dim3(256), 0, st, bp, 6, rowIds,
                       dIA, sbl, dA, dJB, dB, dIC, dJC, dC, err, 0, 0x7fffffff, (int*)nullptr, (double*)nullptr, 0); }
  if (rows(5, 6) > 0) { hipStream_t st = h->side[1]; KTimer t(h, SPGEMM_K_NUM_HASH1, st);
    hipLaunchKernelGGL((k_num64_rows<64, 1024, false>), dim3(clampi(rows(5, 6), 1, cu * 12)), dim3(64), 0, st, bp, 5, rowIds,
                       dIA, sbl, dA, dJB, dB, dIC, dJC, dC, err, 0, 0x7fffffff, (int*)nullptr, (double*)nullptr, 0); }
  if (rows(4, 5) > 0) { hipStream_t st = h->side[0]; KTimer t(h, SPGEMM_K_NUM_G16, st);
    hipLaunchKernelGGL((k_num64_g16<128, 4>), dim3(grid8(cdiv(rows(4, 5), 16), cu * 16)), dim3(256), 0, st, bp, 4, 5, rowIds,
                       dIA, sbl, dA, dJB, dB, dIC, dJC, dC, err, h->rowFlops); }
  if (rows(1, 4) > 0) { KTimer t(h, SPGEMM_K_NUM_SMALL4);
    hipLaunchKernelGGL((k_num64_g16<32, 1>), dim3(grid8(cdiv(rows(1, 4), 16), cu * 16)), dim3(256), 0, s, bp, 1, 4, rowIds,
                       dIA, sbl, dA, dJB, dB, dIC, dJC, dC, err, h->rowFlops); }
  join_streams(h);
  HIPCHK(hipGetLastError());
  return SPGEMM_OK;
}

static int launch_numeric_of(spgemm_handle* h, const int* dIA, const float* dA, const int* dJB, const float* dB, int n,
                             const int* dIC, int* dJC, float* dC, int**) {
  return launch_numeric(h, dIA, dA, dJB, dB, n, h->cur_rowIds, h->mirror.binPtr, dIC, dJC, dC);
}
static int launch_numeric_of(spgemm_handle* h, const int* dIA, const double* dA, const int* dJB, const double* dB, int,
                             const int* dIC, int* dJC, double* dC, int** scratch) {
  return launch_numeric_f64(h, dIA, dA, dJB, dB, h->cur_rowIds, h->mirror.binPtr, dIC, dJC, dC, scratch);
}

template <class V>
static int numeric_phase(spgemm_handle* h, const int* dIA, const int* dJA, const V* dA, const int* dIB, const int* dJB,
                         const V* dB, int m, int n, const int* dIC, int* dJC, V* dC) {
  (void)dJA; (void)dIB;
  constexpr bool isFloat = std::is_same<V, float>::value;
  if (h->sym_m != m) return fail(SPGEMM_ERR_ARG, "numeric phase without a matching symbolic phase on this handle");
  hipStream_t s = h->stream;
  const int nnzC = (int)h->mirror.nnzC64;
  int* scratch[2] = {nullptr, nullptr};
  auto done = [&](int rc) { pool().release(scratch[0]); pool().release(scratch[1]); return rc; };
  hipEventRecord(h->ev[4], s);
  if (m > 0 && nnzC > 0) {
    if (!dJC || !dC) return fail(SPGEMM_ERR_ARG, "output buffers are null");
    if (int rc = launch_numeric_of(h, dIA, dA, dJB, dB, n, dIC, dJC, dC, scratch)) {
      if (!isFloat) (void)hipStreamSynchronize(s);
      return done(rc);
    }
  }
  hipEventRecord(h->ev[5], s);
  if (hipMemcpyAsync(&h->hsmall->err, &h->dsmall->err, sizeof(int), hipMemcpyDeviceToHost, s) != hipSuccess ||
      hipStreamSynchronize(s) != hipSuccess)
    return done(fail(SPGEMM_ERR_HIP, "numeric phase failed: %s", hipGetErrorString(hipGetLastError())));
  h->sym_m = -1;
  if (!(kAblate && isFloat) && h->hsmall->err)
    return done(fail(SPGEMM_ERR_INTERNAL, "device invariant broken in numeric phase (flags=%d)", h->hsmall->err));
  spgemm_stats& st = h->stats;
  hipEventElapsedTime(&st.ms_numeric, h->ev[4], h->ev[5]);
  st.ms_total += st.ms_numeric;
  collect_kernel_times(h, false);
  if (isFloat) { grow_bitmaps(h, n); grow_rehit_log(h, n); }
  return done(SPGEMM_OK);
}

template <class V>
static int finish_exact(spgemm_handle* h, const Product<V>& p, int nnzC, int* dIC, const Result<V>& out) {
  int* dJC = nullptr;
  V* dC = nullptr;
  auto cleanup = [&](int rc) { pool().release(dIC); pool().release(dJC); pool().release(dC); return rc; };
  const size_t cap = (size_t)std::max(nnzC, 1);
  if (hipSuccess != pool().alloc((void**)&dJC, sizeof(int) * cap) || hipSuccess != pool().alloc((void**)&dC, sizeof(V) * cap))
    return cleanup(fail(SPGEMM_ERR_HIP, "device allocation of C (%d entries) failed", nnzC));
  if (int rc = numeric_phase(h, p.IA, p.JA, p.A, p.IB, p.JB, p.B, p.m, p.n, dIC, dJC, dC)) return cleanup(rc);
  *out.IC = dIC; *out.JC = dJC; *out.C = dC; *out.nnz = nnzC;
  return SPGEMM_OK;
}

template <class V>
static int two_phase(spgemm_handle* h, const Product<V>& p, const PreClass* pre, int* dIC, const Result<V>& out) {
  int nnzC = 0;
  if (int rc = symbolic_phase(h, p.IA, p.JA, p.nnzA, p.IB, p.JB, p.m, p.k, p.n, pre, dIC, &nnzC, std::is_same<V, float>::value)) { pool().release(dIC); return rc; }
  return finish_exact(h, p, nnzC, dIC, out);
}

template <class V>
static int begin_product(spgemm_handle** hp, const Product<V>& p, int nnzB, const Result<V>& out, int** dIC) {
  if (!out.IC || !out.JC || !out.C || !out.nnz) return fail(SPGEMM_ERR_ARG, "output pointer is null");
  *out.IC = nullptr; *out.JC = nullptr; *out.C = nullptr; *out.nnz = 0;
  if (p.m < 0 || p.k < 0 || p.n < 0) return fail(SPGEMM_ERR_ARG, "negative dimension m=%d k=%d n=%d", p.m, p.k, p.n);
  CHK(check_common(p.IA, p.JA, p.A, p.nnzA, "A"));
  CHK(check_common(p.IB, p.JB, p.B, nnzB, "B"));
  if (!*hp) CHK(default_handle(hp));
  HIPCHK(hipSetDevice((*hp)->device));
  CHK(ws_ensure(*hp, p.m));
  HIPCHK(pool().alloc((void**)dIC, sizeof(int) * ((size_t)p.m + 1)));
  return SPGEMM_OK;
}

struct OptInPath { bool chain, wb2; int minBin; bool skipH1A; };
static OptInPath opt_in_path(const spgemm_handle* h) {
  const bool chain = h->pathMode == 2, wb2 = h->pathMode == 1;
  return {chain, wb2, (chain || wb2) ? chain_cfg(h).minBin : 0, (chain || wb2) && chain_cfg(h).skipH1A};
}

static int one_shot_front(spgemm_handle* h, const Product<float>& p, const OptInPath& o, int* dIC, HostMirror* mid) {
  hipStream_t s = h->stream;
  hipEventRecord(h->ev[0], s);
  h->cur_rowIds = h->rowIds;
  CHK(launch_classify(h, p.IA, p.JA, p.IB, p.m, p.nnzA, dIC));
  if (o.chain || o.wb2) CHK(launch_cut(h, p.m));
  hipEventRecord(h->ev[1], s);
  if (hipMemcpyAsync(h->hmid, h->dsmall, sizeof(HostMirror), hipMemcpyDeviceToHost, s) != hipSuccess ||
      hipEventRecord(h->evMid, s) != hipSuccess)
    return fail(SPGEMM_ERR_HIP, "classification copy failed: %s", hipGetErrorString(hipGetLastError()));
  if (o.wb2) CHK(launch_wbatch<WB_SYM>(h, p.m, p.IA, nullptr, p.JB, nullptr, dIC, nullptr, nullptr, 0));
  CHK(launch_symbolic(h, p.IA, p.JB, p.m, p.n, h->cur_rowIds, dIC, o.minBin, o.skipH1A, true));
  hipEventRecord(h->ev[2], s);
  if (!o.chain) CHK(launch_scan(h, dIC, p.m, &h->dsmall->nnzC64));
  hipEventRecord(h->ev[3], s);
  if (hipEventSynchronize(h->evMid) != hipSuccess)
    return fail(SPGEMM_ERR_HIP, "classification failed: %s", hipGetErrorString(hipGetLastError()));
  *mid = *h->hmid;
  return SPGEMM_OK;
}

static int one_shot_back(spgemm_handle* h, const Product<float>& p, const OptInPath& o, const HostMirror& mid, size_t capC,
                         int* dIC, const Result<float>& out) {
  const unsigned long long P = mid.totalP;
  hipStream_t s = h->stream;
  int* dJC = nullptr;
  float* dC = nullptr;
  auto cleanup = [&](int rc) { pool().release(dIC); pool().release(dJC); pool().release(dC); return rc; };
  if (hipSuccess != pool().alloc((void**)&dJC, sizeof(int) * capC) || hipSuccess != pool().alloc((void**)&dC, sizeof(float) * capC))
    return cleanup(fail(SPGEMM_ERR_HIP, "device allocation of C (%llu entries) failed", P));
  hipEventRecord(h->ev[4], s);
  h->mirror = mid;
  int rc = SPGEMM_OK;
  if (o.chain) rc = launch_wbatch<WB_CHAIN>(h, p.m, p.IA, p.A, p.JB, p.B, dIC, dJC, dC, (long long)capC);
  if (!rc && o.wb2 && P > 0) rc = launch_wbatch<WB_NUM>(h, p.m, p.IA, p.A, p.JB, p.B, dIC, dJC, dC, (long long)capC);
  if (!rc && P > 0) rc = launch_numeric(h, p.IA, p.A, p.JB, p.B, p.n, h->cur_rowIds, mid.binPtr, dIC, dJC, dC, nullptr, 1, o.minBin, o.skipH1A);
  if (rc) return cleanup(rc);
  hipEventRecord(h->ev[5], s);
  rc = read_mirror(h, "SpGEMM", kAblate ? ~0 : o.chain ? ERRF_CHAIN_CAP : 0);
  if (rc != SPGEMM_ERR_HIP) h->sym_m = -1;
  if (rc) return cleanup(rc);
  const HostMirror& hm = h->mirror;
  if (o.chain && (hm.err & ERRF_CHAIN_CAP)) {
    pool().release(dJC); pool().release(dC);
    h->prev_m = -1; h->prev_nnzC = -1;
    return two_phase(h, p, nullptr, dIC, out);
  }
  publish_stats(h, hm, StatsForm::OneShot);
  grow_bitmaps(h, p.n);
  grow_rehit_log(h, p.n);
  h->prev_m = p.m; h->prev_P = P; h->prev_nnzC = (long long)hm.nnzC64;
  *out.IC = dIC; *out.JC = dJC; *out.C = dC; *out.nnz = (int)hm.nnzC64;
  return SPGEMM_OK;
}

static int spgemm_device(spgemm_handle* h, const Product<float>& p, int nnzB, const PreClass* pre, const Result<float>& out) {
  int* dIC = nullptr;
  CHK(begin_product(&h, p, nnzB, out, &dIC));
  if (pre || p.m == 0) return two_phase(h, p, pre, dIC, out);
  const OptInPath o = opt_in_path(h);
  HostMirror mid;
  int rc = one_shot_front(h, p, o, dIC, &mid);
  if (rc) { pool().release(dIC); return rc; }
  const unsigned long long P = mid.totalP;
  const bool compressive = h->prev_m == p.m && h->prev_P == P && h->prev_nnzC >= 0 && (double)h->prev_nnzC < 0.75 * (double)P;
  if (P <= (1ull << 30) && (!compressive || o.chain)) {
    const size_t capC = compressive ? (size_t)std::max<long long>(h->prev_nnzC, 1ll) : (size_t)std::max<unsigned long long>(P, 1ull);
    return one_shot_back(h, p, o, mid, capC, dIC, out);
  }
  int nnzC = 0;
  rc = o.chain ? symbolic_phase(h, p.IA, p.JA, p.nnzA, p.IB, p.JB, p.m, p.k, p.n, nullptr, dIC, &nnzC)
               : finish_symbolic(h, p.m, &nnzC);
  if (rc) { pool().release(dIC); return rc; }
  h->prev_m = p.m; h->prev_P = P; h->prev_nnzC = nnzC;
  return finish_exact(h, p, nnzC, dIC, out);
}

extern "C" int hip_gpuSpMM(spgemm_handle* h, const int* dIA, const int* dJA, const float* dA, int nnzA,
                           const int* dIB, const int* dJB, const float* dB, int nnzB, int m, int k, int n,
                           int** dIC, int** dJC, float** dC, int* nnzC) {
  return spgemm_device(h, {dIA, dJA, dA, nnzA, dIB, dJB, dB, m, k, n}, nnzB, nullptr, {dIC, dJC, dC, nnzC});
}

extern "C" int hip_spgemm_symbolic(spgemm_handle* h, const int* dIA, const int* dJA, int nnzA, const int* dIB,
                                   const int* dJB, int nnzB, int m, int k, int n, int* dIC, int* nnzC) {
  if (!h) return fail(SPGEMM_ERR_ARG, "hip_spgemm_symbolic needs a handle");
  if (!dIC || !nnzC) return fail(SPGEMM_ERR_ARG, "output pointer is null");
  if (m < 0 || k < 0 || n < 0) return fail(SPGEMM_ERR_ARG, "negative dimension");
  CHK(check_common(dIA, dJA, dJA, nnzA, "A"));
  CHK(check_common(dIB, dJB, dJB, nnzB, "B"));
  HIPCHK(hipSetDevice(h->device));
  CHK(ws_ensure(h, m));
  return symbolic_phase(h, dIA, dJA, nnzA, dIB, dJB, m, k, n, nullptr, dIC, nnzC);
}

extern "C" int hip_spgemm_numeric(spgemm_handle* h, const int* dIA, const int* dJA, const float* dA, int nnzA,
                                  const int* dIB, const int* dJB, const float* dB, int nnzB, int m, int k, int n,
                                  const int* dIC, int* dJC, float* dC) {
  (void)k;
  if (!h) return fail(SPGEMM_ERR_ARG, "hip_spgemm_numeric needs a handle");
  if (!dIC) return fail(SPGEMM_ERR_ARG, "dIC is null");
  CHK(check_common(dIA, dJA, dA, nnzA, "A"));
  CHK(check_common(dIB, dJB, dB, nnzB, "B"));
  HIPCHK(hipSetDevice(h->device));
  return numeric_phase(h, dIA, dJA, dA, dIB, dJB, dB, m, n, dIC, dJC, dC);
}

extern "C" int hip_gpuSpMM_f64(spgemm_handle* h, const int* dIA, const int* dJA, const double* dA, int nnzA,
                               const int* dIB, const int* dJB, const double* dB, int nnzB, int m, int k, int n,
                               int** dICp, int** dJCp, double** dCp, int* nnzCp) {
  const Product<double> p{dIA, dJA, dA, nnzA, dIB, dJB, dB, m, k, n};
  const Result<double> out{dICp, dJCp, dCp, nnzCp};
  int* dIC = nullptr;
  CHK(begin_product(&h, p, nnzB, out, &dIC));
  return two_phase(h, p, nullptr, dIC, out);
}

extern "C" int hip_spgemm_numeric_f64(spgemm_handle* h, const int* dIA, const int* dJA, const double* dA, int nnzA,
                                      const int* dIB, const int* dJB, const double* dB, int nnzB, int m, int k, int n,
                                      const int* dIC, int* dJC, double* dC) {
  (void)k;
  if (!h) return fail(SPGEMM_ERR_ARG, "hip_spgemm_numeric_f64 needs a handle");
  if (!dIC) return fail(SPGEMM_ERR_ARG, "dIC is null");
  CHK(check_common(dIA, dJA, dA, nnzA, "A"));
  CHK(check_common(dIB, dJB, dB, nnzB, "B"));
  HIPCHK(hipSetDevice(h->device));
  return numeric_phase(h, dIA, dJA, dA, dIB, dJB, dB, m, n, dIC, dJC, dC);
}

extern "C" int hip_csr_row_flops(spgemm_handle* h, const int* dIA, const int* dJA, const int* dIB, int m,
                                 int* dRowFlops, long long* total_flops) {
  if (!h) CHK(default_handle(&h));
  if (m < 0 || !dIA || (m > 0 && !dRowFlops)) return fail(SPGEMM_ERR_ARG, "bad argument");
// ... 405 lines not shown
  if (!dIN || !dJN || !dCN || !nnzN) return fail(SPGEMM_ERR_ARG, "output pointer is null");
  *dIN = nullptr; *dJN = nullptr; *dCN = nullptr; *nnzN = 0;
  DevCSR N;
  CHK(rmcl_prune_impl(h, m, nnz, dIC, dJC, dC, &N));
  N.give(dIN, dJN, dCN, nnzN);
  return SPGEMM_OK;
}

extern "C" int hip_rmcl_prune(spgemm_handle* h, int m, const int* dIC, const int* dJC, float* dC, int** dIN, int** dJN,
                              float** dCN, int* nnzN) {
  return rmcl_prune_abi(h, m, -1, dIC, dJC, dC, dIN, dJN, dCN, nnzN);
}

extern "C" int hip_rmcl_prune_n(spgemm_handle* h, int m, int nnz, const int* dIC, const int* dJC, const float* dC,
                                int** dIN, int** dJN, float** dCN, int* nnzN) {
  if (nnz < 0) return fail(SPGEMM_ERR_ARG, "negative nnz");
  return rmcl_prune_abi(h, m, nnz, dIC, dJC, dC, dIN, dJN, dCN, nnzN);
}

static int rmcl_pack_rows(spgemm_handle* h, int m, const CsrView& R, DevCSR* out) {
  out->reset();
  hipStream_t s = h->stream;
  DevCSR N;
  if (N.I.alloc((size_t)m + 1)) return fail(SPGEMM_ERR_NOMEM, "device allocation failed");
  if (hipMemsetAsync(N.I, 0, sizeof(int) * ((size_t)m + 1), s) != hipSuccess ||
      hipMemcpyAsync(N.I, R.len, sizeof(int) * (size_t)m, hipMemcpyDeviceToDevice, s) != hipSuccess)
    return fail(SPGEMM_ERR_HIP, "pack: copy of the row lengths");
  CHK(launch_scan(h, N.I, m, &h->dsmall->kept64));
  if (hipMemcpyAsync(&h->hsmall->kept64, &h->dsmall->kept64, sizeof(unsigned long long), hipMemcpyDeviceToHost, s) != hipSuccess ||
      hipStreamSynchronize(s) != hipSuccess)
    return fail(SPGEMM_ERR_HIP, "pack: scan of the row lengths");
  const unsigned long long total = h->hsmall->kept64;
  if (total > 0x7fffffffULL) return fail(SPGEMM_ERR_OVERFLOW, "pack: %llu entries", total);
  N.nnz = (int)total;
  if (N.alloc_entries(N.nnz)) return fail(SPGEMM_ERR_NOMEM, "device allocation failed");
  if (N.nnz > 0 && m > 0) {
    const RowLanes rl = row_lanes(h, m, 0);
    RMCL_ROWS(k_rmcl_move, rl, s, m, R.I, N.I.p, R.J, R.V, N.J.p, N.V.p);
    if (hipGetLastError() != hipSuccess || hipStreamSynchronize(s) != hipSuccess) return fail(SPGEMM_ERR_HIP, "pack: move");
  }
  *out = std::move(N);
  return SPGEMM_OK;
}

enum { RMCL_EXTENTS = 0, RMCL_PACK = 1, RMCL_BLOCK = 2 };

static int rmcl_hipfail(const char* what) { return fail(SPGEMM_ERR_HIP, "rmcl expand+prune: %s: %s", what, hipGetErrorString(hipGetLastError())); }

static int rmcl_two_steps(spgemm_handle* h, const CsrView& A, CsrView B, int m, int k, int n, DevCSR* out) {
  DevCSR Bp, C;
  if (B.len) { CHK(rmcl_pack_rows(h, k, B, &Bp)); B = Bp.view(); }
  CHK(spgemm_device(h, {A.I, A.J, A.V, A.nnz, B.I, B.J, B.V, m, k, n}, B.nnz, nullptr, {&C.I.p, &C.J.p, &C.V.p, &C.nnz}));
  return rmcl_prune_impl(h, m, C.nnz, C.I, C.J, C.V, out);
}

static int rmcl_classify(spgemm_handle* h, const CsrView& A, const CsrView& B, int m, DevCSR* C, HostMirror* mid, bool* errPending) {
  if (C->I.alloc((size_t)m + 1) || C->len.alloc((size_t)m + 1)) return rmcl_hipfail("device allocation failed");
  hipStream_t s = h->stream;
  h->sym_m = -1;
  hipEventRecord(h->ev[0], s);
  h->cur_rowIds = h->rowIds;
  CHK(launch_classify(h, A.I, A.J, B.I, m, A.nnz, C->I, B.se));
  hipEventRecord(h->ev[1], s);
  if (hipMemcpyAsync(h->hmid, h->dsmall, sizeof(HostMirror), hipMemcpyDeviceToHost, s) != hipSuccess ||
      hipEventRecord(h->evMid, s) != hipSuccess)
    return rmcl_hipfail("classification copy");
  if (hipMemsetAsync(C->len, 0, sizeof(int) * ((size_t)m + 1), s) != hipSuccess) return rmcl_hipfail("memset");
  if (hipEventSynchronize(h->evMid) != hipSuccess) return rmcl_hipfail("classification");
  if (errPending && *errPending) {
    *errPending = false;
    if (h->hsmall->err) return fail(SPGEMM_ERR_INTERNAL, "device invariant broken in the previous iteration (flags=%d)", h->hsmall->err);
  }
  *mid = *h->hmid;
  return SPGEMM_OK;
}

static int rmcl_size_rows_by_products(spgemm_handle* h, const CsrView& A, const CsrView& B, int m, int n, const HostMirror& mid, int* dIC) {
  hipStream_t s = h->stream;
  if (hipMemcpyAsync(dIC, h->rowFlops, sizeof(int) * (size_t)m, hipMemcpyDeviceToDevice, s) != hipSuccess) return rmcl_hipfail("copy");
  const int nbig = mid.binPtr[NBINS] - mid.binPtr[NBINS - 1];
  if (nbig > 0) {
    KTimer t(h, SPGEMM_K_SYM_BIG, s);
    h->bdLogged = false;
    hipLaunchKernelGGL(k_sym_big<false>, dim3(clampi(nbig, 1, h->numCU)), dim3(BIG_THREADS), sizeof(BigSymShared), s,
                       h->dsmall->binPtr, 8, h->cur_rowIds, A.I, h->sbl, B.J, n, dIC, h->bigBitmaps, h->bm_cap,
                       h->dsmall->qctr + 0 * 32, (int2*)nullptr, 0, (int*)nullptr, 0, 0, (int*)nullptr, (int*)nullptr);
    if (hipGetLastError() != hipSuccess) return rmcl_hipfail("symbolic launch");
  }
  return SPGEMM_OK;
}

static int rmcl_numeric(spgemm_handle* h, const CsrView& A, const CsrView& B, int m, int n, const HostMirror& mid, bool nosym,
                        bool scanKept, DevCSR* C) {
  hipStream_t s = h->stream;
  hipEventRecord(h->ev[2], s);
  CHK(launch_scan(h, C->I, m, &h->dsmall->nnzC64));
  hipEventRecord(h->ev[3], s);
  if (C->alloc_entries((long long)mid.totalP)) return rmcl_hipfail("device allocation of the scratch product failed");
  hipEventRecord(h->ev[4], s);
  h->mirror = mid;
  CHK(launch_numeric(h, A.I, A.V, B.J, B.V, n, h->cur_rowIds, mid.binPtr, C->I, C->J, C->V, C->len, nosym ? 2 : 1));
  hipEventRecord(h->ev[5], s);
  return scanKept ? launch_scan(h, C->len, m, &h->dsmall->kept64) : SPGEMM_OK;
}

static int rmcl_leave_extents(spgemm_handle* h, int m, const HostMirror& mid, DevCSR* C) {
  if (C->se.alloc((size_t)m)) return rmcl_hipfail("device allocation failed");
  hipLaunchKernelGGL(k_zip_extents, dim3(cdiv(m, 256)), dim3(256), 0, h->stream, m, C->I.p, C->len.p, C->se.p);
  if (hipGetLastError() != hipSuccess) return rmcl_hipfail("extent launch");
  C->nnz = (int)mid.totalP;
  return SPGEMM_OK;
}

static int rmcl_pack_result(spgemm_handle* h, int m, int nz, DevCSR* C) {
  DevCSR N;
  if (N.alloc_entries(nz)) return rmcl_hipfail("device allocation failed");
  if (nz > 0) {
    const RowLanes rl = row_lanes(h, m, nz);
    RMCL_ROWS(k_rmcl_move, rl, h->stream, m, C->I.p, C->len.p, C->J.p, C->V.p, N.J.p, N.V.p);
    if (hipGetLastError() != hipSuccess) return drained(h->stream, rmcl_hipfail("move launch"));
  }
  if (hipStreamSynchronize(h->stream) != hipSuccess) return drained(h->stream, rmcl_hipfail("move"));
  N.I = std::move(C->len);
  N.nnz = nz;
  *C = std::move(N);
  return SPGEMM_OK;
}

static int rmcl_expand_prune_core(spgemm_handle* h, const CsrView& A, const CsrView& B, int m, int k, int n, int mode,
                                  DevCSR* out, bool* errPending = nullptr) {
  out->reset();
  if (h->failNext > 0) { --h->failNext; return fail(SPGEMM_ERR_INTERNAL, "forced failure (spgemm_hip_debug_fail_next)"); }
  HIPCHK(hipSetDevice(h->device));
  if (m == 0) return rmcl_two_steps(h, A, B, m, k, n, out);
  CHK(ws_ensure(h, m));
  hipStream_t s = h->stream;
  DevCSR C;
  HostMirror mid;
  int rc = rmcl_classify(h, A, B, m, &C, &mid, errPending);
  if (rc) return drained(s, rc);
  unsigned long long maxP = 1ull << 30;
  if (const char* e = getenv("SPGEMM_RMCL_MAXP")) maxP = std::min<unsigned long long>(maxP, strtoull(e, nullptr, 10));
  if (mid.totalP == 0 || mid.totalP > maxP) {
    if (hipStreamSynchronize(s) != hipSuccess) return drained(s, rmcl_hipfail("classification"));
    C.reset();
    return rmcl_two_steps(h, A, B, m, k, n, out);
  }
  const bool nosym = !getenv("SPGEMM_RMCL_SYMBOLIC");
  rc = nosym ? rmcl_size_rows_by_products(h, A, B, m, n, mid, C.I) : launch_symbolic(h, A.I, B.J, m, n, h->cur_rowIds, C.I);
  if (!rc) rc = rmcl_numeric(h, A, B, m, n, mid, nosym, mode != RMCL_EXTENTS, &C);
  if (rc) return drained(s, rc);
  if (mode == RMCL_EXTENTS && errPending && h->ktiming == 0) {
    if (hipMemcpyAsync(h->hsmall, h->dsmall, sizeof(HostMirror), hipMemcpyDeviceToHost, s) != hipSuccess)
      return drained(s, rmcl_hipfail("numeric phase"));
    if ((rc = rmcl_leave_extents(h, m, mid, &C))) return drained(s, rc);
    publish_stats(h, mid, StatsForm::CountsOnly);
    *errPending = true;
    *out = std::move(C);
    return SPGEMM_OK;
  }
  if ((rc = read_mirror(h, "rmcl expand+prune"))) return drained(s, rc);
  publish_stats(h, h->mirror, nosym ? StatsForm::OneShotNoNnz : StatsForm::OneShot);
  grow_bitmaps(h, n);
  const int kept = (int)h->mirror.kept64;
  if (mode == RMCL_BLOCK) C.nnz = kept;
  else if ((rc = mode == RMCL_PACK ? rmcl_pack_result(h, m, kept, &C) : rmcl_leave_extents(h, m, mid, &C))) return drained(s, rc);
// ... 226 lines not shown
```

### sparse_matrix_with_flops_amd/hipspgemm.py

```python
import contextlib
import ctypes as C
import weakref
import os

import numpy as np

_HERE = os.path.dirname(os.path.abspath(__file__))
LIB_PATH = os.environ.get("SPGEMM_LIB") or os.path.join(_HERE, "libspgemm_hip.so")

NBINS = 9
HV_LEN = 9
NKERNELS = 21
_I = C.POINTER(C.c_int)
_F = C.POINTER(C.c_float)
_D = C.POINTER(C.c_double)

EXPORTS = [
    "spgemm_hip_last_error", "spgemm_hip_device_count", "spgemm_hip_create", "spgemm_hip_destroy",
    "spgemm_hip_get_stats", "spgemm_hip_stream", "spgemm_hip_malloc", "spgemm_hip_free",
    "spgemm_hip_memcpy_h2d", "spgemm_hip_memcpy_d2h", "spgemm_hip_memcpy_d2d", "hip_CSR_SpMM", "hip_gpuSpMM",
    "hip_gpuFlopsClassify", "hip_sgpuSpMM", "hip_csr_sort_rows", "spgemm_hip_selftest",
    "hip_spgemm_symbolic", "hip_spgemm_numeric", "hip_csr_row_flops", "spgemm_hip_kernel_name",
    "hip_rmcl_prune", "hip_gpuRmclIter", "hip_coo_to_csr", "hip_flopsStats", "spgemm_hip_set_kernel_timing",
    "hip_rmcl_prune_n", "hip_rmcl_expand_prune", "hip_gpuRmclIter_device", "spgemm_hip_pool_cached_bytes", "hip_nnzStats", "hip_resultsComparison",
    "spgemm_hip_group_create", "spgemm_hip_unique_id", "spgemm_hip_group_create_rank", "spgemm_hip_group_info",
    "spgemm_hip_group_destroy", "hip_sharded_spmm_create", "hip_sharded_spmm_step", "hip_sharded_spmm_result",
    "hip_sharded_spmm_info", "hip_sharded_spmm_destroy", "hip_gpuRmclIter_sharded", "spgemm_hip_host_api_stats",
    "hip_sharded_spmm_handle", "spgemm_hip_rccl_available", "spgemm_hip_pool_trim",
    "hip_sharded_rmcl_create", "hip_sharded_rmcl_run", "hip_sharded_rmcl_continue", "hip_sharded_rmcl_result", "hip_sharded_rmcl_iter_nnz",
    "hip_sharded_rmcl_info", "hip_sharded_rmcl_destroy", "spgemm_hip_debug_fail_next", "spgemm_hip_debug_bigrow_paths", "spgemm_hip_rmcl_devices_used", "spgemm_hip_handle_device",
    "hip_gpuSpMM_f64", "hip_spgemm_numeric_f64", "hip_CSR_SpMM_f64", "hip_csr_sort_rows_f64",
    "hip_csr_permute", "hip_csr_permute_f64", "hip_permutation_transpose", "hip_csr_row_descending_permutation",
    "hip_csr_transpose", "hip_csr_transpose_f64", "spgemm_hip_device_synchronize",
    "hip_csr_diff", "hip_csr_diff_f64", "hip_csr_differsStats", "hip_csr_differsStats_f64",
    "hip_csr_split_columns", "hip_csr_split_columns_f64", "hip_pcsr_join", "hip_pcsr_join_f64",
    "hip_pcsr_spmm", "hip_pcsr_spmm_f64",
    "hip_csr_to_bcsr", "hip_csr_to_bcsr_f64", "hip_bcsr_to_csr", "hip_bcsr_to_csr_f64",
    "hip_csr_to_mcsr", "hip_csr_to_mcsr_f64", "hip_mcsr_to_csr", "hip_mcsr_to_csr_f64",
    "hip_edge_text_header", "hip_parse_edge_lines", "hip_parse_edge_text", "hip_read_edge_file",
]
PCSR_MAX_BLOCKS = 64
BCSR_MAX_TILE = 4096
VALUE_DTYPES = (np.float32, np.float64)
XCHG_AUTO, XCHG_RCCL, XCHG_PEER, XCHG_HOST = 0, 1, 2, 3
XCHG_NAMES = {0: "auto", 1: "rccl", 2: "peer", 3: "host"}
UNIQUE_ID_BYTES = 128


class SpgemmError(RuntimeError):
    pass


class BinReport(C.Structure):
    _fields_ = [("rows", C.c_int), ("rows_differ", C.c_int), ("first_bad_row", C.c_int), ("max_rel_err", C.c_double)]


class CsrDiff(C.Structure):
    _fields_ = [("rows_len_differ", C.c_int), ("first_len_row", C.c_int), ("only_a", C.c_longlong), ("only_b", C.c_longlong),
                ("first_only_row", C.c_int), ("beyond", C.c_longlong), ("first_beyond_row", C.c_int),
                ("max_abs_err", C.c_double), ("max_rel_err", C.c_double), ("max_abs_only_a", C.c_double),
                ("max_abs_only_b", C.c_double), ("sum_sq", C.c_double)]

    def as_dict(self):
        return {name: getattr(self, name) for name, _ in self._fields_}


class EdgeStats(C.Structure):
    _fields_ = [("lines", C.c_longlong), ("first_bad_line", C.c_longlong), ("entries", C.c_int), ("slow_lines", C.c_int),
                ("ms_upload", C.c_float), ("ms_split", C.c_float), ("ms_parse", C.c_float), ("ms_slow", C.c_float),
                ("ms_total", C.c_float)]

    def as_dict(self):
        return {name: getattr(self, name) for name, _ in self._fields_}


class HostApiStats(C.Structure):
    _fields_ = [("ms_h2d", C.c_float), ("ms_device", C.c_float), ("ms_d2h", C.c_float), ("ms_total", C.c_float),
                ("bytes_h2d", C.c_longlong), ("bytes_d2h", C.c_longlong)]


class Stats(C.Structure):
    _fields_ = [("total_flops", C.c_longlong), ("nnzC", C.c_int), ("bin_rows", C.c_int * NBINS),
                ("ms_classify", C.c_float), ("ms_symbolic", C.c_float), ("ms_scan_alloc", C.c_float),
                ("ms_numeric", C.c_float), ("ms_total", C.c_float), ("ms_kernel", C.c_float * NKERNELS)]

    def as_dict(self):
        return {"total_flops": int(self.total_flops), "nnzC": int(self.nnzC), "bin_rows": [int(x) for x in self.bin_rows],
                "ms_classify": float(self.ms_classify), "ms_symbolic": float(self.ms_symbolic),
                "ms_scan_alloc": float(self.ms_scan_alloc), "ms_numeric": float(self.ms_numeric),
                "ms_total": float(self.ms_total),
                "ms_kernel": {kernel_name(i): float(self.ms_kernel[i]) for i in range(NKERNELS)
                              if kernel_name(i) and self.ms_kernel[i] > 0.0}}


_lib = None


def lib():
    global _lib
    if _lib is None:
        if not os.path.exists(LIB_PATH):
            raise SpgemmError(f"{LIB_PATH} is missing: run `make -C sparse_matrix_with_flops_amd/csrc` "
                              "(there is no CPU fallback for the HIP path)")
        L = C.CDLL(LIB_PATH)
        L.spgemm_hip_last_error.restype = C.c_char_p
        L.spgemm_hip_stream.restype = C.c_void_p
        L.spgemm_hip_stream.argtypes = [C.c_void_p]
        L.spgemm_hip_create.argtypes = [C.POINTER(C.c_void_p), C.c_int]
        L.spgemm_hip_destroy.argtypes = [C.c_void_p]
        L.spgemm_hip_get_stats.argtypes = [C.c_void_p, C.POINTER(Stats)]
        L.spgemm_hip_malloc.argtypes = [C.POINTER(C.c_void_p), C.c_size_t]
        L.spgemm_hip_free.argtypes = [C.c_void_p]
        L.spgemm_hip_memcpy_h2d.argtypes = [C.c_void_p, C.c_void_p, C.c_size_t]
# ... 27 lines not shown
        L.hip_gpuRmclIter_device.argtypes = [C.c_void_p, C.c_int, C.c_int, C.c_int] + dev_in + dev_in + \
            [C.POINTER(C.c_void_p)] * 3 + [C.POINTER(C.c_int)]
        L.hip_rmcl_prune_n.argtypes = [C.c_void_p, C.c_int, C.c_int, C.c_void_p, C.c_void_p, C.c_void_p] + \
            [C.POINTER(C.c_void_p)] * 3 + [_I]
        L.spgemm_hip_pool_cached_bytes.argtypes = [C.c_int, C.POINTER(C.c_size_t)]
        L.hip_nnzStats.argtypes = [C.c_void_p, C.c_void_p, C.c_int, C.POINTER(C.c_int)]
        L.hip_resultsComparison.argtypes = [C.c_int, C.c_int, _I, _I, _F, _I, _I, _F, _I, C.c_int, _I, C.c_double,
                                            C.POINTER(BinReport)]
        L.hip_gpuRmclIter.argtypes = [C.c_int, C.c_int, C.c_int, _I, _I, _F, C.c_int, _I, _I, _F, C.c_int,
                                      C.POINTER(_I), C.POINTER(_I), C.POINTER(_F), _I]
        L.hip_csr_sort_rows.argtypes = [C.c_void_p, C.c_int, C.c_void_p, C.c_void_p, C.c_void_p]
        L.hip_CSR_SpMM_f64.argtypes = [_I, _I, _D, C.c_int, _I, _I, _D, C.c_int, C.POINTER(_I), C.POINTER(_I),
                                       C.POINTER(_D), _I, C.c_int, C.c_int, C.c_int]
        L.hip_gpuSpMM_f64.argtypes = L.hip_gpuSpMM.argtypes
        L.hip_spgemm_numeric_f64.argtypes = L.hip_spgemm_numeric.argtypes
        L.hip_csr_sort_rows_f64.argtypes = L.hip_csr_sort_rows.argtypes
        L.hip_csr_permute.argtypes = [C.c_void_p, C.c_int, C.c_int, C.c_int, C.c_void_p, C.c_void_p, C.c_void_p,
                                      C.c_void_p, C.c_void_p] + [C.POINTER(C.c_void_p)] * 3
        L.hip_csr_permute_f64.argtypes = L.hip_csr_permute.argtypes
        L.hip_permutation_transpose.argtypes = [C.c_void_p, C.c_int, C.c_void_p, C.c_void_p]
        L.hip_csr_row_descending_permutation.argtypes = [C.c_void_p, C.c_int, C.c_void_p, C.POINTER(C.c_void_p)]
        L.hip_csr_transpose.argtypes = [C.c_void_p, C.c_int, C.c_int, C.c_int, C.c_void_p, C.c_void_p, C.c_void_p] + \
            [C.POINTER(C.c_void_p)] * 3
        L.hip_csr_transpose_f64.argtypes = L.hip_csr_transpose.argtypes
        L.hip_csr_diff.argtypes = [C.c_void_p, C.c_int, C.c_int] + dev_in + dev_in + [C.c_double, C.c_double,
                                                                                          C.POINTER(CsrDiff)]
        L.hip_csr_diff_f64.argtypes = L.hip_csr_diff.argtypes
        L.hip_csr_differsStats.argtypes = [C.c_void_p, C.c_int, C.c_void_p, C.c_void_p, _F, C.c_int, _I]
        L.hip_csr_differsStats_f64.argtypes = [C.c_void_p, C.c_int, C.c_void_p, C.c_void_p, _D, C.c_int, _I]
        table = [C.POINTER(C.c_void_p)] * 3 + [_I]
        L.hip_csr_split_columns.argtypes = [C.c_void_p, C.c_int, C.c_int, C.c_int, C.c_void_p, C.c_void_p, C.c_void_p,
                                            C.c_int] + [C.POINTER(C.c_void_p)] * 3 + [_I]
        L.hip_csr_split_columns_f64.argtypes = L.hip_csr_split_columns.argtypes
        L.hip_pcsr_join.argtypes = [C.c_void_p, C.c_int, C.c_int, C.c_int] + table + [C.POINTER(C.c_void_p)] * 3 + [_I]
        L.hip_pcsr_join_f64.argtypes = L.hip_pcsr_join.argtypes
        L.hip_pcsr_spmm.argtypes = [C.c_void_p] + dev_in + [C.c_int, C.c_int, C.c_int, C.c_int] + table + table
        L.hip_pcsr_spmm_f64.argtypes = L.hip_pcsr_spmm.argtypes
        L.hip_csr_to_bcsr.argtypes = [C.c_void_p, C.c_int, C.c_int, C.c_int, C.c_void_p, C.c_void_p, C.c_void_p, C.c_int,
                                      C.c_int] + [C.POINTER(C.c_void_p)] * 3 + [_I]
        L.hip_csr_to_bcsr_f64.argtypes = L.hip_csr_to_bcsr.argtypes
        L.hip_bcsr_to_csr.argtypes = [C.c_void_p, C.c_int, C.c_int, C.c_int, C.c_int, C.c_int, C.c_void_p, C.c_void_p,
                                      C.c_void_p, C.c_double] + [C.POINTER(C.c_void_p)] * 3 + [_I]
        L.hip_bcsr_to_csr_f64.argtypes = L.hip_bcsr_to_csr.argtypes
        L.hip_csr_to_mcsr.argtypes = [C.c_void_p, C.c_int, C.c_int, C.c_int, C.c_void_p, C.c_void_p, C.c_void_p, C.c_int,
                                      C.c_int, C.c_int, C.c_int] + ([C.POINTER(C.c_void_p)] * 3 + [_I]) * 2
        L.hip_csr_to_mcsr_f64.argtypes = L.hip_csr_to_mcsr.argtypes
        L.hip_mcsr_to_csr.argtypes = [C.c_void_p] + [C.c_int] * 6 + [C.c_int, C.c_void_p, C.c_void_p, C.c_void_p] * 2 + \
            [C.c_double] + [C.POINTER(C.c_void_p)] * 3 + [_I]
        L.hip_mcsr_to_csr_f64.argtypes = L.hip_mcsr_to_csr.argtypes
        L.hip_edge_text_header.argtypes = [C.c_char_p, C.c_size_t, _I, _I, _I, _I, _I, C.POINTER(C.c_size_t)]
        edge_out = [C.POINTER(C.c_void_p)] * 3 + [_I, C.POINTER(EdgeStats)]
        L.hip_parse_edge_lines.argtypes = [C.c_void_p, C.c_void_p, C.c_size_t, C.c_int, C.c_int] + edge_out
        L.hip_parse_edge_text.argtypes = [C.c_void_p, C.c_char_p, C.c_size_t, C.c_int, C.c_int] + edge_out
        L.hip_read_edge_file.argtypes = [C.c_void_p, C.c_char_p, C.c_int, C.c_int, _I, _I] + edge_out
        L.spgemm_hip_selftest.argtypes = [C.c_void_p]
        L.spgemm_hip_set_kernel_timing.argtypes = [C.c_void_p, C.c_uint]
        host_in = [_I, _I, _F, C.c_int]
        L.spgemm_hip_host_api_stats.argtypes = [C.POINTER(HostApiStats)]
        L.spgemm_hip_group_create.argtypes = [C.POINTER(C.c_void_p), C.c_int, _I, C.c_int]
        L.spgemm_hip_unique_id.argtypes = [C.c_void_p]
        L.spgemm_hip_group_create_rank.argtypes = [C.POINTER(C.c_void_p), C.c_int, C.c_int, C.c_int, C.c_void_p]
        L.spgemm_hip_group_info.argtypes = [C.c_void_p, _I, _I, _I]
        L.spgemm_hip_group_destroy.argtypes = [C.c_void_p]
        L.hip_sharded_spmm_create.argtypes = [C.c_void_p] + host_in + host_in + [C.c_int, C.c_int, C.c_int,
                                                                                   C.POINTER(C.c_void_p)]
        L.hip_sharded_spmm_step.argtypes = [C.c_void_p, C.c_int, C.POINTER(C.c_longlong), C.POINTER(C.c_longlong)]
        L.hip_sharded_spmm_result.argtypes = [C.c_void_p, C.c_int, C.POINTER(_I), C.POINTER(_I), C.POINTER(_F), _I, _I]
        L.hip_sharded_spmm_info.argtypes = [C.c_void_p, _I, C.POINTER(C.c_float), C.POINTER(C.c_float)]
        L.hip_sharded_spmm_destroy.argtypes = [C.c_void_p]
        L.hip_sharded_spmm_handle.argtypes = [C.c_void_p, C.c_int]
        L.hip_sharded_spmm_handle.restype = C.c_void_p
        L.hip_gpuRmclIter_sharded.argtypes = [C.c_void_p, C.c_int, C.c_int, C.c_int] + host_in + host_in + \
            [C.POINTER(_I), C.POINTER(_I), C.POINTER(_F), _I]
        L.hip_sharded_rmcl_create.argtypes = [C.c_void_p, C.c_int, C.c_int] + host_in + host_in + [C.POINTER(C.c_void_p)]
        L.hip_sharded_rmcl_run.argtypes = [C.c_void_p, C.c_int, _I]
        L.hip_sharded_rmcl_continue.argtypes = [C.c_void_p, C.c_int, _I]
        L.hip_sharded_rmcl_result.argtypes = [C.c_void_p, C.c_int, C.POINTER(_I), C.POINTER(_I), C.POINTER(_F), _I]
        L.hip_sharded_rmcl_iter_nnz.argtypes = [C.c_void_p, C.POINTER(C.c_longlong), C.c_int]
        L.hip_sharded_rmcl_info.argtypes = [C.c_void_p, _I]
        L.hip_sharded_rmcl_destroy.argtypes = [C.c_void_p]
        L.spgemm_hip_debug_fail_next.argtypes = [C.c_void_p, C.c_int]
        if hasattr(L, "spgemm_hip_debug_bigrow_paths"):
            L.spgemm_hip_debug_bigrow_paths.argtypes = [C.c_void_p] + [C.POINTER(C.c_int)] * 4
        L.spgemm_hip_handle_device.argtypes = [C.c_void_p]
        L.free = C.CDLL(None).free
        L.free.argtypes = [C.c_void_p]
        _lib = L
    return _lib


def kernel_name(i):
    return lib().spgemm_hip_kernel_name(int(i)).decode()


def _check(rc, what):
    if rc != 0:
        raise SpgemmError(f"{what} failed with status {rc}: {lib().spgemm_hip_last_error().decode(errors='replace')}")


def device_count():
    n = C.c_int(0)
    rc = lib().spgemm_hip_device_count(C.byref(n))
    return n.value if rc == 0 else 0


def _typed(name, dtype):
    name = name + "_f64" if _value_dtype(dtype) == np.float64 else name
    return getattr(lib(), name), name


def _call(name, dtype, *args):
    fn, name = _typed(name, dtype)
    _check(fn(*args), name)


def _hp(handle):
    return handle.ptr if handle else None


def _ptrs(*device_pointers):
    return [C.c_void_p(p) for p in device_pointers]


class _CsrOut:

    def __init__(self, count=True):
        self._slots = [C.c_void_p(), C.c_void_p(), C.c_void_p()] + ([C.c_int(0)] if count else [])

    def refs(self):
        return [C.byref(s) for s in self._slots]

    def values(self):
        return tuple(s.value for s in self._slots)


_LIVE = weakref.WeakSet()


def _close_all():
    live = list(_LIVE)
    for kind in ("ShardedSpMM", "ShardedRmcl", "Group", "Handle"):
        for o in live:
            if type(o).__name__ == kind:
                try:
                    o.close()
                except Exception:
                    pass


import atexit
atexit.register(_close_all)


class Handle:

    def __init__(self, device=0, _borrowed=None):
        self._own = _borrowed is None
        if _borrowed is not None:
            self._h = C.c_void_p(_borrowed)
        else:
            self._h = C.c_void_p()
            _check(lib().spgemm_hip_create(C.byref(self._h), int(device)), "spgemm_hip_create")
            _LIVE.add(self)
        self.device = device if _borrowed is None else int(lib().spgemm_hip_handle_device(self._h))

    @property
    def ptr(self):
        return self._h

    def stats(self):
        s = Stats()
        _check(lib().spgemm_hip_get_stats(self._h, C.byref(s)), "spgemm_hip_get_stats")
        return s.as_dict()

    def stream(self):
        return lib().spgemm_hip_stream(self._h)

    def selftest(self):
        _check(lib().spgemm_hip_selftest(self._h), "spgemm_hip_selftest")

    def set_kernel_timing(self, mask):
        _check(lib().spgemm_hip_set_kernel_timing(self._h, int(mask) & 0xFFFFFFFF), "spgemm_hip_set_kernel_timing")

    def fail_next(self, count=1):
        _check(lib().spgemm_hip_debug_fail_next(self._h, int(count)), "spgemm_hip_debug_fail_next")

    def bigrow_paths(self):
        v = [C.c_int(0) for _ in range(4)]
        _check(lib().spgemm_hip_debug_bigrow_paths(self._h, *[C.byref(x) for x in v]), "spgemm_hip_debug_bigrow_paths")
        return {"direct": v[0].value, "fallback": v[1].value, "cap": v[2].value, "region": v[3].value}

    def close(self):
        if self._h and self._own:
            lib().spgemm_hip_destroy(self._h)
        self._h = C.c_void_p()

    def __del__(self):
        try:
            self.close()
        except Exception:
            pass


def dev_alloc(nbytes):
    p = C.c_void_p()
    _check(lib().spgemm_hip_malloc(C.byref(p), max(int(nbytes), 1)), "spgemm_hip_malloc")
    return p.value


def dev_free(ptr):
    if ptr:
        _check(lib().spgemm_hip_free(C.c_void_p(ptr)), "spgemm_hip_free")


def h2d(arr):
    arr = np.ascontiguousarray(arr)
    p = dev_alloc(arr.nbytes)
    if arr.nbytes:
        _check(lib().spgemm_hip_memcpy_h2d(C.c_void_p(p), arr.ctypes.data_as(C.c_void_p), arr.nbytes), "h2d")
    return p


def d2h(ptr, n, dtype):
    out = np.empty(int(n), dtype=dtype)
    if out.nbytes:
        _check(lib().spgemm_hip_memcpy_d2h(out.ctypes.data_as(C.c_void_p), C.c_void_p(ptr), out.nbytes), "d2h")
    return out


class CSR:

    def __init__(self, values=None, colInd=None, rowPtr=None, rows=0, cols=0, nnz=0, on_device=False, dtype=None):
        self.values, self.colInd, self.rowPtr = values, colInd, rowPtr
        self.rows, self.cols, self.nnz = int(rows), int(cols), int(nnz)
        self.on_device = on_device
        if dtype is None:
            dtype = values.dtype if isinstance(values, np.ndarray) else np.float32
        self.dtype = np.dtype(dtype)

    @staticmethod
    def from_arrays(rowPtr, colInd, values, rows, cols, dtype=np.float32):
        dtype = _value_dtype(dtype)
        rowPtr = np.ascontiguousarray(rowPtr, dtype=np.int32)
        return CSR(np.ascontiguousarray(values, dtype=dtype), np.ascontiguousarray(colInd, dtype=np.int32),
                   rowPtr, rows, cols, int(rowPtr[-1]) if len(rowPtr) else 0, dtype=dtype)

    def toGpuCSR(self):
        assert not self.on_device
        return CSR(h2d(self.values), h2d(self.colInd), h2d(self.rowPtr), self.rows, self.cols, self.nnz, True,
                   dtype=self.dtype)

    def toCpuCSR(self):
        assert self.on_device
        return CSR(d2h(self.values, self.nnz, self.dtype), d2h(self.colInd, self.nnz, np.int32),
                   d2h(self.rowPtr, self.rows + 1, np.int32), self.rows, self.cols, self.nnz, False, dtype=self.dtype)

    def deviceDispose(self):
        assert self.on_device
        for p in (self.values, self.colInd, self.rowPtr):
            dev_free(p)
        self.values = self.colInd = self.rowPtr = None

    def makeOrdered(self):
        assert not self.on_device
        row_of = np.repeat(np.arange(self.rows, dtype=np.int64), np.diff(self.rowPtr.astype(np.int64)))
        order = np.lexsort((self.colInd, row_of))
        self.colInd = np.ascontiguousarray(self.colInd[order])
        self.values = np.ascontiguousarray(self.values[order])

    def hip_spmm(self, B):
        assert not self.on_device and not B.on_device
        if self.cols != B.rows:
            raise SpgemmError(f"shape mismatch: A is {self.rows}x{self.cols}, B is {B.rows}x{B.cols}")
# ... 971 lines not shown
```

Baseline: 179.3 GFLOP/s.

## Log mid-bin rehit columns in symbolic pass to enable direct numeric kernel

Result: faster. 185.9 GFLOP/s (median of 6 runs) (+3.7%).

```diff
diff --git a/include/spgemm_hip.h b/include/spgemm_hip.h
--- a/include/spgemm_hip.h
+++ b/include/spgemm_hip.h
@@ -167,6 +167,9 @@
 int spgemm_hip_debug_fail_next(spgemm_handle* h, int count);
 
 int spgemm_hip_debug_bigrow_paths(spgemm_handle* h, int* direct_rows, int* fallback_rows, int* rehit_cap, int* region_ints);
+
+int spgemm_hip_debug_midrow_paths(spgemm_handle* h, int* rows, int* direct_rows, int* fallback_rows, int* rehit_cap);
+int spgemm_hip_debug_midrow_log(spgemm_handle* h, long long* logged, long long* reserved, long long* capacity);
 
 #define SPGEMM_COO_DEDUPE         1
 #define SPGEMM_COO_SELF_LOOPS     2
diff --git a/sparse_matrix_with_flops_amd/csrc/spgemm_device.hpp b/sparse_matrix_with_flops_amd/csrc/spgemm_device.hpp
--- a/sparse_matrix_with_flops_amd/csrc/spgemm_device.hpp
+++ b/sparse_matrix_with_flops_amd/csrc/spgemm_device.hpp
@@ -133,9 +133,9 @@
 
 constexpr int DUMMY_KEY = (int)0x80000000;
 
-template <bool POW2 = true, int U>
+template <bool POW2 = true, bool RH = false, int U>
 __device__ __forceinline__ int hash_insert_multi(int* keys, int size, int shift, const bool (&act)[U],
-                                                 const int (&col)[U], int* dummy, int* err) {
+                                                 const int (&col)[U], int* dummy, int* err, bool (*rehit)[U] = nullptr) {
   char* const base = reinterpret_cast<char*>(keys);
   const int dumB = (int)(reinterpret_cast<char*>(dummy) - base);
   const int maskB = size * 4 - 1;
@@ -146,6 +146,7 @@
     const unsigned hv = (unsigned)col[u] * 2654435761u;
     const unsigned h = POW2 ? hv >> shift : __umulhi(hv, (unsigned)size);
     hB[u] = act[u] ? (int)(h * 4u) : dumB;
+    if constexpr (RH) (*rehit)[u] = false;
   }
   int probe = 0;
   for (;;) {
@@ -157,6 +158,7 @@
 #pragma unroll
     for (int u = 0; u < U; ++u) {
       claimed += old[u] == EMPTY_KEY ? 1 : 0;
+      if constexpr (RH) (*rehit)[u] = (*rehit)[u] || old[u] == col[u];
       const bool adv = hB[u] != dumB && old[u] != EMPTY_KEY && old[u] != col[u];
       const int nh = POW2 ? ((hB[u] + probe * 4) & maskB) : (hB[u] + 4 == size * 4 ? 0 : hB[u] + 4);
       hB[u] = adv ? nh : dumB;
@@ -260,19 +262,23 @@
 }
 
 template <int NW> struct InsChunk { static constexpr int value = NW == 1 ? 1 : 0; };
-template <int CH, int R>
+template <int CH, bool RH = false, int R>
 __device__ __forceinline__ int hash_insert_chunked(int* keys, int size, int shift, const bool (&act)[R], const int (&col)[R],
-                                                   int* dummy, int* err) {
-  if constexpr (CH <= 0 || CH >= R) return hash_insert_multi(keys, size, shift, act, col, dummy, err);
+                                                   int* dummy, int* err, bool (*rehit)[R] = nullptr) {
+  if constexpr (CH <= 0 || CH >= R) return hash_insert_multi<true, RH>(keys, size, shift, act, col, dummy, err, rehit);
   else {
     int claimed = 0;
 #pragma unroll
     for (int c0 = 0; c0 < R; c0 += CH) {
-      bool a_[CH]; int c_[CH];
-#pragma unroll
-      for (int u = 0; u < CH; ++u) { a_[u] = c0 + u < R ? act[c0 + u < R ? c0 + u : 0] : false; c_[u] = col[c0 + u < R ? c0 + u : 0]; }
-      if (CH == 1 && ballot64(a_[0]) == 0ull) continue;
-      claimed += hash_insert_multi(keys, size, shift, a_, c_, dummy, err);
+      bool a_[CH]; int c_[CH]; bool r_[CH];
+#pragma unroll
+      for (int u = 0; u < CH; ++u) { a_[u] = c0 + u < R ? act[c0 + u < R ? c0 + u : 0] : false; c_[u] = col[c0 + u < R ? c0 + u : 0]; r_[u] = false; }
+      if (!(CH == 1 && ballot64(a_[0]) == 0ull))
+        claimed += hash_insert_multi<true, RH>(keys, size, shift, a_, c_, dummy, err, RH ? &r_ : nullptr);
+      if constexpr (RH) {
+#pragma unroll
+        for (int u = 0; u < CH; ++u) if (c0 + u < R) (*rehit)[c0 + u] = r_[u];
+      }
     }
     return claimed;
   }
@@ -1116,17 +1122,35 @@
   return p;
 }
 
-template <int NW, int TBL, int U>
+constexpr int MD_CHUNK = 4096;
+struct MidLogArgs {
+  int2* meta;
+  int* log;
+  long long logCap;
+  int cap;
+  unsigned long long* cursor;
+  int* fbList;
+  int* fbCount;
+  unsigned long long* logged;
+};
+
+template <int NW, int TBL, int U, bool LOG = false>
 __global__ __launch_bounds__(WAVE * NW) void k_sym_hash(const int* __restrict__ binPtr, int bin,
                                                          const int* __restrict__ rowIds,
                                                          const int* __restrict__ IA, const int2* __restrict__ SBL,
                                                          const int* __restrict__ JB,
                                                          const int* __restrict__ rowFlops, int* __restrict__ IC,
-                                                         int* __restrict__ err, int* __restrict__ qctr) {
+                                                         int* __restrict__ err, int* __restrict__ qctr, MidLogArgs ml) {
+  static_assert(!LOG || NW > 1, "only the multi-wave kernels log");
   __shared__ __attribute__((aligned(16))) int keys[TBL];
   __shared__ typename WalkSel<NW>::type st;
   __shared__ int cnt_s;
   __shared__ int qslot;
+  __shared__ int logCnt_s, logOvf_s;
+  __shared__ unsigned long long chunk_s;
+  unsigned long long chunkStart = 0ull;
+  int cursor = MD_CHUNK;
+  unsigned long long loggedSum = 0ull;
   const int tid = threadIdx.x, lane = lane_id();
   if (tid < WAVE) st.dummy[tid] = DUMMY_SLOT;
   int first = binPtr[bin], count = binPtr[bin + 1] - first;
@@ -1157,11 +1181,47 @@
     const int shift = 32 - log2_pow2(size);
     clear_table(keys, nullptr, size, tid, WAVE * NW);
     if (tid == 0) cnt_s = 0;
+    const bool newChunk = LOG && cursor + ml.cap > MD_CHUNK;
+    if constexpr (LOG) if (tid == 0) {
+      logCnt_s = 0; logOvf_s = 0;
+      if (newChunk) chunk_s = atomicAdd(ml.cursor, (unsigned long long)MD_CHUNK);
+    }
     __syncthreads();
+    if constexpr (LOG) if (newChunk) { chunkStart = chunk_s; cursor = 0; }
+    const bool logging = LOG && chunkStart + (unsigned long long)MD_CHUNK <= (unsigned long long)ml.logCap;
+    int* const myLog = LOG && logging ? ml.log + chunkStart + cursor : nullptr;
+    const int room = LOG ? min(ml.cap, MD_CHUNK - cursor) : 0;
     int mine = 0;
     for_each_product<NW, U, false>(st, cur.as, cur.ae, SBL, nullptr, JB, nullptr,
                                    [&](const auto& act, const auto& col, const auto& val, int) {
+      if constexpr (!LOG)
       mine += hash_insert_chunked<InsChunk<NW>::value>(keys, size, shift, act, col, reinterpret_cast<int*>(&st.dummy[lane_id()]), err);
+      else {
+        constexpr int R = (int)(sizeof(col) / sizeof(col[0]));
+        bool rehit[R];
+        mine += hash_insert_chunked<InsChunk<NW>::value, true>(keys, size, shift, act, col,
+                                                               reinterpret_cast<int*>(&st.dummy[lane_id()]), err, &rehit);
+        if (logging) {
+          unsigned long long mk[R];
+          int tot = 0;
+#pragma unroll
+          for (int u = 0; u < R; ++u) { mk[u] = ballot64(rehit[u]); tot += __popcll(mk[u]); }
+          if (tot) {
+            int base = 0;
+            if (lane_id() == 0) base = atomicAdd(&logCnt_s, tot);
+            base = __builtin_amdgcn_readfirstlane(base);
+            if (base + tot > room) {
+              if (lane_id() == 0) logOvf_s = 1;
+            } else {
+#pragma unroll
+              for (int u = 0; u < R; ++u) {
+                if (rehit[u]) myLog[base + mask_rank(mk[u])] = col[u];
+                base += __popcll(mk[u]);
+              }
+            }
+          }
+        }
+      }
     }, pc, err);
     const int ws = wave_sum(mine);
     if (NW == 1) {
@@ -1170,12 +1230,24 @@
       if (lane == 0 && ws) atomicAdd(&cnt_s, ws);
       __syncthreads();
       if (tid == 0) IC[cur.row] = cnt_s;
+      if constexpr (LOG) {
+        const int logged = logCnt_s;
+        const int rehits = cur.x0 - cnt_s;
+        const bool direct = logging && !logOvf_s;
+        if (tid == 0) {
+          ml.meta[cur.row] = make_int2((int)chunkStart + cursor, direct ? logged : -1);
+          if (!direct) ml.fbList[atomicAdd(ml.fbCount, 1)] = cur.row;
+        }
+        if (direct) { cursor += logged; loggedSum += (unsigned long long)logged; }
+        else if (!logging && rehits >= 0 && rehits <= ml.cap) cursor += rehits;
+      }
     }
     __syncthreads();
     cur = nxt;
     if (NW == 1) { nxt = nn; pc = pn; }
     q = qn;
   }
+  if constexpr (LOG) if (tid == 0 && loggedSum) atomicAdd(ml.logged, loggedSum);
 }
 
 template <int NW, int TBL, int U, int PRUNE = 0>
@@ -1907,6 +1979,157 @@
   }
 }
 
+#ifndef SMF_MD_U
+#define SMF_MD_U 4
+#endif
+constexpr int MD_U = SMF_MD_U;
+template <int NW, int S>
+struct MidDirectShared {
+  slot_t tab[S];
+  WalkStageN<NW> st;
+  int qslot;
+  int emitted;
+};
+struct MidMeta { RowMeta m; int ls, lc; };
+__device__ __forceinline__ MidMeta load_meta_mid(const int* rows, int q, int count, const int* IA, const int* IC,
+                                                 const int* rowFlops, const int2* meta, int cap) {
+  MidMeta d{{0, 0, 0, 0, 0, 0}, 0, -1};
+  if (q < count) {
+    const int row = rows[q];
+    const int2 lm = meta[row];
+    if (lm.y >= 0 && lm.y <= cap) { d.ls = lm.x; d.lc = lm.y; d.m = load_meta_num(rows, q, count, IA, IC, rowFlops); }
+  }
+  return d;
+}
+
+template <int NW, int S>
+__global__ __launch_bounds__(WAVE * NW) void k_num_middirect(const int* __restrict__ binPtr, int bin,
+                                                             const int* __restrict__ rowIds,
+                                                             const int* __restrict__ IA, const int2* __restrict__ SBL,
+                                                             const float* __restrict__ VA,
+                                                             const int* __restrict__ JB,
+                                                             const float* __restrict__ VB,
+                                                             const int* __restrict__ IC, int* __restrict__ JC,
+                                                             float* __restrict__ C, int* __restrict__ err,
+                                                             int* __restrict__ qctr, const int* __restrict__ rowFlops,
+                                                             const int2* __restrict__ meta, const int* __restrict__ mlog,
+                                                             long long logCap, int cap) {
+  constexpr int T = WAVE * NW;
+  static_assert(S % T == 0 && S / T <= 8, "every wave sweeps whole 64-slot steps");
+  static_assert(sizeof(WalkNumber<NW>) <= S * sizeof(slot_t), "the numbering of an expanded row lives in the table");
+  __shared__ __attribute__((aligned(16))) MidDirectShared<NW, S> sh;
+  const int tid = threadIdx.x, lane = lane_id(), w = tid >> 6;
+  const int first = binPtr[bin], count = binPtr[bin + 1] - first;
+  const int* rows = rowIds + first;
+  cap = min(cap, bd_cap(S));
+  if (tid < WAVE) sh.st.dummy[tid] = DUMMY_SLOT;
+  constexpr int QB = NW >= 8 ? 2 : 4;
+  int q = next_row<QB>(qctr, &sh.qslot, -1);
+  MidMeta cur = load_meta_mid(rows, q, count, IA, IC, rowFlops, meta, cap);
+  while (q < count) {
+    const int qn = next_row<QB>(qctr, &sh.qslot, q);
+    const MidMeta nxt = load_meta_mid(rows, qn, count, IA, IC, rowFlops, meta, cap);
+    const int as = cur.m.as, ae = cur.m.ae;
+    const int outBase = cur.m.x0, outEnd = cur.m.x1;
+    const int want = outEnd - outBase;
+    int* const JCrow = JC + outBase;
+    float* const Crow = C + outBase;
+    const unsigned lim = (unsigned)max(want, 0);
+    const bool mine = cur.lc >= 0 && (long long)cur.ls >= 0 && (long long)cur.ls + cur.lc <= logCap;
+    if (mine && want == cur.m.x2) {
+      for_each_product<NW, MD_U, true>(sh.st, as, ae, SBL, VA, JB, VB,
+                                       [&](const bool (&act)[MD_U], const int (&col)[MD_U], const float (&val)[MD_U], int p0) {
+#pragma unroll
+        for (int u = 0; u < MD_U; ++u) {
+          const unsigned o = (unsigned)(p0 + u * WAVE + lane);
+          if (act[u] && o < lim) { st_out(JCrow + o, col[u]); st_out(Crow + o, val[u]); }
+        }
+      }, PreA{0, 0, 0.f, false}, err, reinterpret_cast<WalkNumber<NW>*>(sh.tab));
+    } else if (mine) {
+      const int lc = cur.lc;
+      const int size = table_size<4>(lc, T, S);
+      const int shift = 32 - log2_pow2(size);
+      const int per = size / NW;
+      clear_slots(sh.tab, size, tid, T);
+      if (tid == 0) sh.emitted = 0;
+      __syncthreads();
+      {
+        const int* const lg = mlog + cur.ls;
+        const unsigned mask = (unsigned)size - 1u;
+        for (int i = tid; i < lc; i += T) {
+          const int c = lg[i];
+          const slot_t own = make_slot(c, -0.0f);
+          unsigned h = ((unsigned)c * 2654435761u) >> shift;
+          for (int probe = 0; probe < size; ++probe) {
+            const slot_t old = atomicCAS(&sh.tab[h], EMPTY_SLOT, own);
+            if (old == EMPTY_SLOT || slot_key(old) == c) break;
+            h = (h + 1u) & mask;
+          }
+        }
+      }
+      __syncthreads();
+      for_each_product<NW, MD_U, true>(sh.st, as, ae, SBL, VA, JB, VB,
+                                       [&](const bool (&act)[MD_U], const int (&col)[MD_U], const float (&val)[MD_U], int) {
+        char* const base = reinterpret_cast<char*>(sh.tab);
+        const int dumB = (int)(reinterpret_cast<char*>(&sh.st.dummy[lane]) - base);
+        const int maskB = size * 8 - 1;
+        int hB[MD_U], hitB[MD_U];
+        bool miss[MD_U];
+#pragma unroll
+        for (int u = 0; u < MD_U; ++u) {
+          const unsigned h = ((unsigned)col[u] * 2654435761u) >> shift;
+          hB[u] = act[u] ? (int)(h * 8u) : dumB;
+          hitB[u] = dumB;
+          miss[u] = false;
+        }
+        for (int probe = 0;;) {
+          int key[MD_U];
+#pragma unroll
+          for (int u = 0; u < MD_U; ++u) key[u] = *reinterpret_cast<const int*>(base + hB[u]);
+          ++probe;
+          int pendBits = 0;
+#pragma unroll
+          for (int u = 0; u < MD_U; ++u) {
+            const bool pend = hB[u] != dumB;
+            const bool hit = pend && key[u] == col[u];
+            const bool emp = pend && key[u] == EMPTY_KEY;
+            hitB[u] = hit ? hB[u] : hitB[u];
+            miss[u] = miss[u] || emp;
+            hB[u] = (pend && !hit && !emp) ? ((hB[u] + 8) & maskB) : dumB;
+            pendBits |= hB[u] ^ dumB;
+          }
+          if (ballot64(pendBits != 0) == 0ull) break;
+          if (probe >= size) { atomicOr(err, ERRF_TABLE_FULL); break; }
+        }
+#pragma unroll
+        for (int u = 0; u < MD_U; ++u)
+          if (hitB[u] != dumB) atomicAdd(reinterpret_cast<float*>(base + hitB[u] + 4), val[u]);
+        unsigned long long mk[MD_U];
+        int tot = 0;
+#pragma unroll
+        for (int u = 0; u < MD_U; ++u) { mk[u] = ballot64(miss[u]); tot += __popcll(mk[u]); }
+        if (tot) {
+          int pos = 0;
+          if (lane == 0) pos = atomicAdd(&sh.emitted, tot);
+          pos = __builtin_amdgcn_readfirstlane(pos);
+#pragma unroll
+          for (int u = 0; u < MD_U; ++u) {
+            const unsigned o = (unsigned)(pos + mask_rank(mk[u]));
+            if (miss[u] && o < lim) { st_out(JCrow + o, col[u]); st_out(Crow + o, val[u]); }
+            pos += __popcll(mk[u]);
+          }
+        }
+      });
+      emit_claimed<S / T>(sh.tab, w * per, per, &sh.emitted, outBase, outEnd, JC, C);
+      __syncthreads();
+      if (tid == 0 && sh.emitted != want) atomicOr(err, ERRF_COUNT_MISMATCH);
+      __syncthreads();
+    }
+    cur = nxt;
+    q = qn;
+  }
+}
+
 constexpr int SCAN_THREADS = 1024;
 constexpr int SCAN_ITEMS = 4;
 constexpr int SCAN_TILE = SCAN_THREADS * SCAN_ITEMS;
diff --git a/sparse_matrix_with_flops_amd/csrc/spgemm_hip.hip b/sparse_matrix_with_flops_amd/csrc/spgemm_hip.hip
--- a/sparse_matrix_with_flops_amd/csrc/spgemm_hip.hip
+++ b/sparse_matrix_with_flops_amd/csrc/spgemm_hip.hip
@@ -174,7 +174,7 @@
   int binPtr[NBINS + 1];
   int err;
   int scratch2[4];
-  alignas(128) int qctr[9 * 32];
+  alignas(128) int qctr[10 * 32];
   alignas(128) int qpad_;
   int slotBase[NSLOTS + 1];
   unsigned long long totalP;
@@ -185,6 +185,9 @@
   alignas(128) int chainTicket;
   alignas(128) int chainPad_;
   alignas(128) int fbBin[2];
+  alignas(128) int fbMid[4];
+  alignas(128) unsigned long long mrCursor;
+  unsigned long long mrLogged[2];
   alignas(128) int fbPad_;
 };
 
@@ -240,6 +243,17 @@
   int* bigFallback = nullptr;
   bool bdLogged = false;
   bool bdRan = false;
+  bool midDirect = true;
+  int mdCfg = -1;
+  int mdCap = 0;
+  int mdMinRows = 0;
+  long long mrLogEnv = 0;
+  int2* mrMeta = nullptr;
+  int* midFallback = nullptr;
+  int* mrLog = nullptr;
+  long long mr_cap = 0;
+  bool mdLogged = false;
+  bool mdRan[2] = {false, false};
   int h1sym = 32;
   int h1num = 24;
   spgemm_stats stats;
@@ -254,7 +268,7 @@
 static std::map<int, int> g_handles_on;
 
 struct WsBlock { void** ptr; size_t bytes; };
-static std::array<WsBlock, 10> ws_blocks(spgemm_handle* h, size_t cap) {
+static std::array<WsBlock, 12> ws_blocks(spgemm_handle* h, size_t cap) {
   const size_t nblk = (cap + K1_THREADS - 1) / K1_THREADS;
   const size_t ntile = (cap + 1 + SCAN_TILE - 1) / SCAN_TILE + 1;
   return {{{(void**)&h->rowFlops, sizeof(int) * cap},
@@ -265,6 +279,8 @@
            {(void**)&h->tileSum, sizeof(unsigned long long) * ntile},
            {(void**)&h->blockP, sizeof(unsigned long long) * nblk},
            {(void**)&h->bigFallback, sizeof(int) * cap},
+           {(void**)&h->mrMeta, sizeof(int2) * cap},
+           {(void**)&h->midFallback, sizeof(int) * 2 * cap},
            {(void**)&h->batchStart, sizeof(int) * (3 * cap + 64)},
            {(void**)&h->chainWords, sizeof(unsigned long long) * (3 * cap + 64)}}};
 }
@@ -307,6 +323,18 @@
   }
 }
 static int bd_cap_of(int cfg) { return bd_cap(cfg == 2 || cfg == 3 ? 8192 : 4096); }
+template <class F>
+static auto with_md_cfg(int cfg, F f) {
+  typedef std::integral_constant<int, 4> W4; typedef std::integral_constant<int, 8> W8;
+  typedef std::integral_constant<int, 1024> S1; typedef std::integral_constant<int, 2048> S2;
+  switch (cfg) {
+    case 1: return f(W8(), S1());
+    case 2: return f(W4(), S2());
+    case 3: return f(W8(), S2());
+    default: return f(W4(), S1());
+  }
+}
+static int md_slots_of(int cfg) { return cfg >= 2 ? 2048 : 1024; }
 
 static void env_int(const char* name, int lo, int hi, int* field) {
   if (const char* e = getenv(name)) { const int v = atoi(e); if (v >= lo && v <= hi) *field = v; }
@@ -351,6 +379,13 @@
   h->bdMinRows = h->numCU;
   env_int("SPGEMM_BD_MINROWS", 1, 1 << 30, &h->bdMinRows);
   env_int("SPGEMM_RLREGION", 64, 1 << 24, &h->rlRegionEnv);
+  { int v = 1; env_int("SPGEMM_MIDDIRECT", 0, 1, &v); h->midDirect = v != 0; }
+  env_int("SPGEMM_MD_CFG", 0, 3, &h->mdCfg);
+  h->mdCap = bd_cap(md_slots_of(h->mdCfg));
+  env_int("SPGEMM_MD_CAP", 0, h->mdCap, &h->mdCap);
+  h->mdMinRows = 4 * h->numCU;
+  env_int("SPGEMM_MD_MINROWS", 1, 1 << 30, &h->mdMinRows);
+  { int v = 0; env_int("SPGEMM_MRLOG", 1, 1 << 30, &v); h->mrLogEnv = v; }
   env_int("SPGEMM_PATH", 0, 2, &h->pathMode);
   env_int("SPGEMM_CHAIN_CFG", INT_MIN, INT_MAX, &h->chainCfg);
   { int u = h->U; env_int("SPGEMM_U", 2, 8, &u); if (u == 2 || u == 4 || u == 8) h->U = u; }
@@ -388,6 +423,7 @@
   hipFree(h->spill);
   hipFree(h->rlMeta);
   hipFree(h->rlLog);
+  hipFree(h->mrLog);
   hipFree(h->sbl);
   hipFree(h->dsmall);
   hipHostFree(h->hsmall);
@@ -422,6 +458,24 @@
   *direct_rows = nbig - *fallback_rows;
   *rehit_cap = bd_cap_of(h->bdCfg);
   *region_ints = h->rl_region;
+  return SPGEMM_OK;
+}
+
+extern "C" int spgemm_hip_debug_midrow_paths(spgemm_handle* h, int* rows, int* direct_rows, int* fallback_rows, int* rehit_cap) {
+  if (!h || !rows || !direct_rows || !fallback_rows || !rehit_cap) return fail(SPGEMM_ERR_ARG, "null argument");
+  *rows = h->mirror.binPtr[8] - h->mirror.binPtr[6];
+  *fallback_rows = 0;
+  for (int b = 0; b < 2; ++b) *fallback_rows += h->mdRan[b] ? h->mirror.fbMid[2 * b + 1] : h->mirror.binPtr[7 + b] - h->mirror.binPtr[6 + b];
+  *direct_rows = *rows - *fallback_rows;
+  *rehit_cap = h->mdCap;
+  return SPGEMM_OK;
+}
+extern "C" int spgemm_hip_debug_midrow_log(spgemm_handle* h, long long* logged, long long* reserved, long long* capacity) {
+  if (!h || !logged || !reserved || !capacity) return fail(SPGEMM_ERR_ARG, "null argument");
+  *logged = 0;
+  for (int b = 0; b < 2; ++b) if (h->mdRan[b]) *logged += (long long)h->mirror.mrLogged[b];
+  *reserved = h->mdLogged ? (long long)h->mirror.mrCursor : 0;
+  *capacity = h->mr_cap;
   return SPGEMM_OK;
 }
 
@@ -604,6 +658,7 @@
                            int m, int n, const int* rowIds, int* dIC, int minBin = 0, bool skipH1A = false, bool logBig = false) {
   const int2* sbl = h->sbl;
   h->bdLogged = logBig && h->bigDirect && n > BIG_WC && m > 0;
+  h->mdLogged = logBig && h->midDirect && m > 0 && minBin == 0 && h->pathMode == 0 && h->U == 2;
   if (m <= 0) return SPGEMM_OK;
   clear_stale_hip_error();
   const int* bp = h->dsmall->binPtr;
@@ -621,19 +676,31 @@
       hipLaunchKernelGGL(k_sym_big<false>, dim3(clampi(m, 1, cu)), dim3(BIG_THREADS), sizeof(BigSymShared), st, bp, 8,
                          rowIds, dIA, sbl, dJB, n, dIC, h->bigBitmaps, h->bm_cap, qc + 0 * 32,
                          (int2*)nullptr, 0, (int*)nullptr, 0, 0, (int*)nullptr, (int*)nullptr); }
+  auto mid_log = [&](int which) {
+    return MidLogArgs{h->mrMeta, h->mrLog, h->mrLog ? h->mr_cap : 0ll, h->mdCap, &h->dsmall->mrCursor,
+                      h->midFallback + (which ? h->cap_m : 0), &h->dsmall->fbMid[2 * which + 1], &h->dsmall->mrLogged[which]};
+  };
   if (minBin <= 7) { hipStream_t st = h->side[2]; KTimer t(h, SPGEMM_K_SYM_HASH8, st);
+    if (h->mdLogged)
+      hipLaunchKernelGGL((k_sym_hash<8, 8192, 2, true>), dim3(clampi(m, 1, cu * 3)), dim3(512), 0, st, bp, 7, rowIds, dIA,
+                         sbl, dJB, h->rowFlops, dIC, err, qc + 1 * 32, mid_log(1));
+    else
     LAUNCH_U(k_sym_hash, 8, 8192, dim3(clampi(m, 1, cu * 3)), dim3(512), st, bp, 7, rowIds, dIA,
-             sbl, dJB, h->rowFlops, dIC, err, qc + 1 * 32); }
+             sbl, dJB, h->rowFlops, dIC, err, qc + 1 * 32, MidLogArgs{}); }
   if (minBin <= 6) { hipStream_t st = h->side[2]; KTimer t(h, SPGEMM_K_SYM_HASH4, st);
+    if (h->mdLogged)
+      hipLaunchKernelGGL((k_sym_hash<4, 4096, 2, true>), dim3(clampi(m, 1, cu * 8)), dim3(256), 0, st, bp, 6, rowIds, dIA,
+                         sbl, dJB, h->rowFlops, dIC, err, qc + 2 * 32, mid_log(0));
+    else
     LAUNCH_U(k_sym_hash, 4, 4096, dim3(clampi(m, 1, cu * 8)), dim3(256), st, bp, 6, rowIds, dIA,
-             sbl, dJB, h->rowFlops, dIC, err, qc + 2 * 32); }
+             sbl, dJB, h->rowFlops, dIC, err, qc + 2 * 32, MidLogArgs{}); }
   if (minBin <= 5) { hipStream_t st = h->side[1]; KTimer t(h, SPGEMM_K_SYM_HASH1, st);
     const int* sb = h->dsmall->slotBase;
     if (!skipH1A)
     LAUNCH_U(k_sym_hash, 1, 512, dim3(grid8(m, cu * h->h1sym)), dim3(64), st, sb, SLOT_H1A, rowIds, dIA,
-             sbl, dJB, h->rowFlops, dIC, err, qc + 3 * 32);
+             sbl, dJB, h->rowFlops, dIC, err, qc + 3 * 32, MidLogArgs{});
     LAUNCH_U(k_sym_hash, 1, 1024, dim3(grid8(m, cu * h->h1sym)), dim3(64), st, sb, SLOT_H1B, rowIds, dIA,
-             sbl, dJB, h->rowFlops, dIC, err, qc + 3 * 32); }
+             sbl, dJB, h->rowFlops, dIC, err, qc + 3 * 32, MidLogArgs{}); }
   if (minBin <= 4) { hipStream_t st = h->side[0]; KTimer t(h, SPGEMM_K_SYM_G16, st);
     hipLaunchKernelGGL((k_sym_g16<128, 4>), dim3(grid8(cdiv(m, 16), cu * 16)), dim3(256), 0, st, bp, 4, 5,
                        rowIds, dIA, sbl, dJB, h->rowFlops, dIC, err); }
@@ -700,10 +767,30 @@
     if (pcnt) hipLaunchKernelGGL(k_rmcl_fix_rows, dim3(clampi(rows(8, 9), 1, cu * 8)), dim3(256), 0, st,
                                  bp, 8, 9, rowIds, dIC, dJC, dC, pcnt);
   }
-  if (rows(7, 8) > 0) { hipStream_t st = h->side[2]; KTimer t(h, SPGEMM_K_NUM_HASH8, st);
+  const bool mid = h->mdLogged && h->mrLog && !pcnt && minBin <= 6;
+  const bool mid6 = mid && rows(6, 7) >= h->mdMinRows, mid7 = mid && rows(7, 8) >= h->mdMinRows;
+  h->mdRan[0] = mid6; h->mdRan[1] = mid7;
+  auto launch_mid = [&](int bin, int nrows, int* qd, hipStream_t st) {
+    with_md_cfg(h->mdCfg >= 0 ? h->mdCfg : bin == 7 ? 1 : 0, [&](auto nw, auto slots) {
+      const int lds = (int)sizeof(MidDirectShared<nw, slots>);
+      const int perCU = std::max(1, std::min((160 * 1024) / lds, 32 / (int)nw));
+      hipLaunchKernelGGL((k_num_middirect<nw, slots>), dim3(clampi(nrows, 1, cu * perCU)), dim3(WAVE * nw), 0, st,
+                         bp, bin, rowIds, dIA, sbl, dA, dJB, dB, dIC, dJC, dC, err, qd, (const int*)h->rowFlops,
+                         (const int2*)h->mrMeta, (const int*)h->mrLog, h->mr_cap, h->mdCap);
+      return 0; });
+  };
+  if (mid7) { hipStream_t st = h->side[2]; KTimer t(h, SPGEMM_K_NUM_HASH8, st);
+    launch_mid(7, rows(7, 8), qc + 9 * 32, st);
+    LAUNCH_U(k_num_hash, 8, 8192, dim3(clampi(rows(7, 8), 1, cu * 2)), dim3(512), st, h->dsmall->fbMid + 2, 0,
+             (const int*)(h->midFallback + h->cap_m), dIA, sbl, dA, dJB, dB, dIC, dJC, dC, err, qc + 5 * 32, h->rowFlops, (int*)nullptr); }
+  if (mid6) { hipStream_t st = h->side[2]; KTimer t(h, SPGEMM_K_NUM_HASH4, st);
+    launch_mid(6, rows(6, 7), qc + 6 * 32, st);
+    LAUNCH_U(k_num_hash, 4, 4096, dim3(clampi(rows(6, 7), 1, cu * 4)), dim3(256), st, h->dsmall->fbMid, 0,
+             (const int*)h->midFallback, dIA, sbl, dA, dJB, dB, dIC, dJC, dC, err, qc + 7 * 32, h->rowFlops, (int*)nullptr); }
+  if (!mid7 && rows(7, 8) > 0) { hipStream_t st = h->side[2]; KTimer t(h, SPGEMM_K_NUM_HASH8, st);
     LAUNCH_NUM(8, 8192, dim3(clampi(rows(7, 8), 1, cu * 2)), dim3(512), st, bp, 7,
              rowIds, dIA, sbl, dA, dJB, dB, dIC, dJC, dC, err, qc + 5 * 32, h->rowFlops); }
-  if (rows(6, 7) > 0) { hipStream_t st = h->side[2]; KTimer t(h, SPGEMM_K_NUM_HASH4, st);
+  if (!mid6 && rows(6, 7) > 0) { hipStream_t st = h->side[2]; KTimer t(h, SPGEMM_K_NUM_HASH4, st);
     const int* sb = h->dsmall->slotBase;
     const int* hs_ = h->mirror.slotBase;
     const int na = hs_[SLOT_H4A + 1] - hs_[SLOT_H4A], nb = hs_[SLOT_H4B + 1] - hs_[SLOT_H4B];
@@ -908,6 +995,18 @@
     hipFree(h->rlMeta); hipFree(h->rlLog);
     h->rlMeta = nullptr; h->rlLog = nullptr;
   }
+}
+
+static void grow_midrow_log(spgemm_handle* h) {
+  const int* hb = h->mirror.binPtr;
+  if (!h->mdLogged || std::max(hb[7] - hb[6], hb[8] - hb[7]) < h->mdMinRows) return;
+  const long long used = (long long)std::min<unsigned long long>(h->mirror.mrCursor, 1ull << 30);
+  if (used == 0 || (h->mrLog && (h->mrLogEnv > 0 || used <= h->mr_cap))) return;
+  hipFree(h->mrLog);
+  h->mrLog = nullptr; h->mr_cap = 0;
+  const long long want = h->mrLogEnv > 0 ? h->mrLogEnv : std::min<long long>(used + used / 4 + 16 * MD_CHUNK, 1ll << 30);
+  if (hipMalloc((void**)&h->mrLog, (size_t)want * sizeof(int)) == hipSuccess) h->mr_cap = want;
+  else (void)hipGetLastError();
 }
 
 static int launch_numeric_f64(spgemm_handle* h, const int* dIA, const double* dA, const int* dJB, const double* dB,
@@ -1012,7 +1111,7 @@
   hipEventElapsedTime(&st.ms_numeric, h->ev[4], h->ev[5]);
   st.ms_total += st.ms_numeric;
   collect_kernel_times(h, false);
-  if (isFloat) { grow_bitmaps(h, n); grow_rehit_log(h, n); }
+  if (isFloat) { grow_bitmaps(h, n); grow_rehit_log(h, n); grow_midrow_log(h); }
   return done(SPGEMM_OK);
 }
 
@@ -1106,6 +1205,7 @@
   publish_stats(h, hm, StatsForm::OneShot);
   grow_bitmaps(h, p.n);
   grow_rehit_log(h, p.n);
+  grow_midrow_log(h);
   h->prev_m = p.m; h->prev_P = P; h->prev_nnzC = (long long)hm.nnzC64;
   *out.IC = dIC; *out.JC = dJC; *out.C = dC; *out.nnz = (int)hm.nnzC64;
   return SPGEMM_OK;
@@ -1677,6 +1777,7 @@
   if (nbig > 0) {
     KTimer t(h, SPGEMM_K_SYM_BIG, s);
     h->bdLogged = false;
+    h->mdLogged = false;
     hipLaunchKernelGGL(k_sym_big<false>, dim3(clampi(nbig, 1, h->numCU)), dim3(BIG_THREADS), sizeof(BigSymShared), s,
                        h->dsmall->binPtr, 8, h->cur_rowIds, A.I, h->sbl, B.J, n, dIC, h->bigBitmaps, h->bm_cap,
                        h->dsmall->qctr + 0 * 32, (int2*)nullptr, 0, (int*)nullptr, 0, 0, (int*)nullptr, (int*)nullptr);
diff --git a/sparse_matrix_with_flops_amd/hipspgemm.py b/sparse_matrix_with_flops_amd/hipspgemm.py
--- a/sparse_matrix_with_flops_amd/hipspgemm.py
+++ b/sparse_matrix_with_flops_amd/hipspgemm.py
@@ -28,7 +28,7 @@
     "hip_sharded_spmm_info", "hip_sharded_spmm_destroy", "hip_gpuRmclIter_sharded", "spgemm_hip_host_api_stats",
     "hip_sharded_spmm_handle", "spgemm_hip_rccl_available", "spgemm_hip_pool_trim",
     "hip_sharded_rmcl_create", "hip_sharded_rmcl_run", "hip_sharded_rmcl_continue", "hip_sharded_rmcl_result", "hip_sharded_rmcl_iter_nnz",
-    "hip_sharded_rmcl_info", "hip_sharded_rmcl_destroy", "spgemm_hip_debug_fail_next", "spgemm_hip_debug_bigrow_paths", "spgemm_hip_rmcl_devices_used", "spgemm_hip_handle_device",
+    "hip_sharded_rmcl_info", "hip_sharded_rmcl_destroy", "spgemm_hip_debug_fail_next", "spgemm_hip_debug_bigrow_paths", "spgemm_hip_debug_midrow_paths", "spgemm_hip_debug_midrow_log", "spgemm_hip_rmcl_devices_used", "spgemm_hip_handle_device",
     "hip_gpuSpMM_f64", "hip_spgemm_numeric_f64", "hip_CSR_SpMM_f64", "hip_csr_sort_rows_f64",
     "hip_csr_permute", "hip_csr_permute_f64", "hip_permutation_transpose", "hip_csr_row_descending_permutation",
     "hip_csr_transpose", "hip_csr_transpose_f64", "spgemm_hip_device_synchronize",
@@ -222,6 +222,9 @@
         L.spgemm_hip_debug_fail_next.argtypes = [C.c_void_p, C.c_int]
         if hasattr(L, "spgemm_hip_debug_bigrow_paths"):
             L.spgemm_hip_debug_bigrow_paths.argtypes = [C.c_void_p] + [C.POINTER(C.c_int)] * 4
+        if hasattr(L, "spgemm_hip_debug_midrow_paths"):
+            L.spgemm_hip_debug_midrow_paths.argtypes = [C.c_void_p] + [C.POINTER(C.c_int)] * 4
+            L.spgemm_hip_debug_midrow_log.argtypes = [C.c_void_p] + [C.POINTER(C.c_longlong)] * 3
         L.spgemm_hip_handle_device.argtypes = [C.c_void_p]
         L.free = C.CDLL(None).free
         L.free.argtypes = [C.c_void_p]
@@ -329,6 +332,14 @@
         v = [C.c_int(0) for _ in range(4)]
         _check(lib().spgemm_hip_debug_bigrow_paths(self._h, *[C.byref(x) for x in v]), "spgemm_hip_debug_bigrow_paths")
         return {"direct": v[0].value, "fallback": v[1].value, "cap": v[2].value, "region": v[3].value}
+
+    def midrow_paths(self):
+        v = [C.c_int(0) for _ in range(4)]
+        w = [C.c_longlong(0) for _ in range(3)]
+        _check(lib().spgemm_hip_debug_midrow_paths(self._h, *[C.byref(x) for x in v]), "spgemm_hip_debug_midrow_paths")
+        _check(lib().spgemm_hip_debug_midrow_log(self._h, *[C.byref(x) for x in w]), "spgemm_hip_debug_midrow_log")
+        return {"rows": v[0].value, "direct": v[1].value, "fallback": v[2].value, "cap": v[3].value,
+                "logged": w[0].value, "reserved": w[1].value, "capacity": w[2].value}
 
     def close(self):
         if self._h and self._own:
```
